# david-m-rosen/Optimization

Measured on AMD Instinct MI355X. Metric: TNT Steihaug-CG HVP+inner-product throughput, higher is better.
Workload: dtype f64

## Files before the change

include/mi355opt.h:

```cpp
#ifndef MI355OPT_H
#define MI355OPT_H

#include <stddef.h>
#include <stdint.h>

#ifdef __cplusplus
extern "C" {
#endif

#define MI_API __attribute__((visibility("default")))

typedef enum mi_status {
  MI_OK = 0,
  MI_ERR_INVALID_ARGUMENT = 1,
  MI_ERR_HIP = 2,
  MI_ERR_OOM = 3,
  MI_ERR_NO_DEVICE = 4,
  MI_ERR_COMM = 5,
  MI_ERR_INTERNAL = 6,
  MI_DECLINED = 7
} mi_status;

typedef struct mi_ctx mi_ctx;
typedef struct mi_vec mi_vec;
// ... 196 lines not shown
MI_API int mi_stiefel_retract(mi_ctx *ctx, size_t n, int p, const mi_vec *X, const mi_vec *V,
                              mi_vec *Y);
MI_API int mi_stiefel_rq_create(mi_ctx *ctx, const mi_csr *A, size_t n, int p, mi_stiefel_rq **out);
MI_API int mi_stiefel_rq_destroy(mi_stiefel_rq *prob);
MI_API int mi_stiefel_rq_objective(mi_stiefel_rq *prob, const mi_vec *X, double *f);
MI_API int mi_stiefel_rq_model(mi_stiefel_rq *prob, const mi_vec *X, mi_vec *grad, mi_op **hess);
MI_API int mi_stiefel_rq_trial(mi_stiefel_rq *prob, const mi_vec *X, const mi_vec *h, const mi_vec *g,
                               mi_vec *X_trial, double out[5]);
MI_API int mi_stiefel_rq_armijo_trial(mi_stiefel_rq *prob, const mi_vec *X, const mi_vec *g, double t, mi_vec *h_out,
                                      mi_vec *X_trial, double out[2]);
MI_API int mi_stiefel_rq_precon(mi_stiefel_rq *prob, const mi_vec *X, const mi_vec *dinv_rows,
                                mi_precon **out);

MI_API int mi_so3n_create(mi_ctx *ctx, size_t N, size_t n_edges, const int32_t *ei,
                          const int32_t *ej, const double *Rt , const double *w,
                          mi_so3n **out);
MI_API int mi_so3n_destroy(mi_so3n *prob);
MI_API int mi_so3n_objective(mi_so3n *prob, const mi_vec *R, double *f);
MI_API int mi_so3n_model(mi_so3n *prob, const mi_vec *R, mi_vec *grad, mi_op **hess,
                         mi_precon **block_jacobi );
MI_API int mi_so3n_retract(mi_so3n *prob, const mi_vec *R, const mi_vec *xi, mi_vec *Y);
MI_API int mi_so3n_trial(mi_so3n *prob, const mi_vec *R, const mi_vec *h, const mi_vec *g, int with_precon,
                         mi_vec *R_trial, double out[6]);

MI_API int mi_lobpcg_gram(mi_ctx *ctx, size_t m, int ka, int kb, const mi_vec *S, const mi_vec *AS,
                          double *G_host);
MI_API int mi_lobpcg_gram_split(mi_ctx *ctx, size_t m, int k, const mi_vec *S, int k1, const mi_vec *T1,
                                const mi_vec *T2, double *G_host);
MI_API int mi_lobpcg_gram_pair(mi_ctx *ctx, size_t m, int k, const mi_vec *S, int k1a, const mi_vec *Ta1,
                               const mi_vec *Ta2, int k1b, const mi_vec *Tb1, const mi_vec *Tb2, double *Ga_host,
                               double *Gb_host);
MI_API int mi_lobpcg_gram_pair_sym(mi_ctx *ctx, size_t m, int k, const mi_vec *S, int k1a, const mi_vec *Ta1,
                                   const mi_vec *Ta2, double *Ga_host, double *Gb_host);
typedef struct mi_panel_blocks {
  int nblocks;
  const mi_vec *block[3];
  int cols[3];
} mi_panel_blocks;
MI_API int mi_lobpcg_gram_pair_sym_blocks(mi_ctx *ctx, size_t m, const mi_panel_blocks *S, int k1a, const mi_vec *Ta1,
                                          const mi_vec *Ta2, double *Ga_host, double *Gb_host);
MI_API int mi_lobpcg_gram_pair_sym_tblocks(mi_ctx *ctx, size_t m, const mi_panel_blocks *S, const mi_panel_blocks *T,
                                           double *Ga_host, double *Gb_host);
MI_API int mi_lobpcg_gram_pair_gen_blocks(mi_ctx *ctx, size_t m, const mi_panel_blocks *S, const mi_panel_blocks *AS,
                                          const mi_panel_blocks *BS, double *Ga_host, double *Gb_host);
MI_API int mi_lobpcg_update2_blocks(mi_ctx *ctx, size_t m, const mi_panel_blocks *S, int kc, const double *C_host,
                                    int ldc, mi_vec *Y, int k1, mi_vec *Y2);
MI_API int mi_csr_spmm_colmajor_blocks(const mi_csr *A, const mi_panel_blocks *X, mi_vec *Y);
MI_API int mi_lobpcg_update(mi_ctx *ctx, size_t m, int ks, int kc, const mi_vec *S,
                            const double *C_host, int ldc, mi_vec *Y);
MI_API int mi_lobpcg_update2(mi_ctx *ctx, size_t m, int ks, int kc, const mi_vec *S, const double *C_host, int ldc,
                             mi_vec *Y, int k1, mi_vec *Y2);
MI_API int mi_lobpcg_residual(mi_ctx *ctx, size_t m, int nx, const mi_vec *AX, const mi_vec *BX,
                              const mi_vec *X, const double *theta_host, mi_vec *R, double *rnorm,
                              double *xnorm);
MI_API int mi_rayleigh_ritz(int n, const double *A, const double *B, double *Theta, double *C);
MI_API int mi_rayleigh_ritz_lowest(int n, int k, const double *A, const double *B, double *Theta, double *C);
MI_API int mi_csr_spmm_colmajor(const mi_csr *A, int k, const mi_vec *X, mi_vec *Y);
MI_API int mi_csr_spmm_colmajor_residual(const mi_csr *A, int nx, const mi_vec *X, const double *theta_host,
                                         mi_vec *AX, mi_vec *R, double *rnorm, double *xnorm);
MI_API int mi_panel_rowscale(mi_ctx *ctx, size_t m, int k, const mi_vec *d, const mi_vec *X, mi_vec *Y);

#define MI_COMM_UID_BYTES 128
MI_API int mi_comm_unique_id(unsigned char uid[MI_COMM_UID_BYTES]);
MI_API int mi_comm_init(mi_ctx *ctx, int world_size, int rank,
                        const unsigned char uid[MI_COMM_UID_BYTES]);
MI_API int mi_comm_finalize(mi_ctx *ctx);
MI_API int mi_comm_info(mi_ctx *ctx, int *world_size, int *rank);
MI_API int mi_comm_rccl_count(mi_ctx *ctx, int *nranks);
#define MI_COMM_IPC_HANDLE_BYTES 64
MI_API int mi_comm_ipc_export(mi_ctx *ctx, unsigned char handle[MI_COMM_IPC_HANDLE_BYTES]);
MI_API int mi_comm_ipc_attach(mi_ctx *ctx, int world_size, int rank,
                              const unsigned char *handles );
MI_API int mi_comm_ipc_selftest(mi_ctx *ctx, int *ok);
MI_API int mi_comm_ipc_enable(mi_ctx *ctx, int on);
MI_API int mi_comm_ipc_error(mi_ctx *ctx, int *err);
MI_API int mi_comm_ipc_fold(mi_ctx *ctx, int on);
MI_API int mi_comm_kernel_launches(mi_ctx *ctx, unsigned long long out[4]);
MI_API int mi_debug_csr_window_info(const mi_csr *A, size_t out[4]);
MI_API int mi_debug_csr_format_info(const mi_csr *A, size_t out[5]);
MI_API int mi_debug_so3n_info(const mi_so3n *q, size_t out[6]);
MI_API int mi_debug_window_runs(int ntiles, int max_wgs, int num_cu, size_t far_stride, int *bounds_out, int cap,
                                int *nb_out);
MI_API int mi_debug_stiefel_hess_form(int p, int gram_count, const size_t traits[9], const int switches[9], int out[14]);
MI_API int mi_debug_set_rank(mi_ctx *ctx, int world_size, int rank);
MI_API int mi_debug_csr_set_halo(mi_csr *A, int p, const double *halo_rows_host);
MI_API int mi_debug_time_fused_apply(mi_op *op, const mi_vec *in, mi_vec *out, int reps, double *us_per_call);
MI_API int mi_csr_shard_plan(size_t n_global, int world_size, int rank, const size_t *row_starts,
                             size_t nnz_local, const int64_t *col_global, int32_t *col_local, size_t *need_lo,
                             size_t *need_hi);
MI_API int mi_csr_create_sharded(mi_ctx *ctx, size_t n_global, size_t row_begin, size_t row_end,
                                 size_t nnz_local, const int32_t *rowptr, const int64_t *col_global,
                                 const double *val, const size_t *row_starts ,
                                 mi_csr **out);

#ifdef __cplusplus
}
#endif
#endif
```

optimization_amd/capi.py:

```python
import ctypes as C
import os

import numpy as np

_HERE = os.path.dirname(os.path.abspath(__file__))
LIB_PATH = os.environ.get("MI355OPT_LIB") or os.path.join(_HERE, "libmi355opt.so")

MI_OK = 0
STATUS = {0: "MI_OK", 1: "MI_ERR_INVALID_ARGUMENT", 2: "MI_ERR_HIP", 3: "MI_ERR_OOM",
          4: "MI_ERR_NO_DEVICE", 5: "MI_ERR_COMM", 6: "MI_ERR_INTERNAL", 7: "MI_DECLINED"}
KERNELS = ["none", "cg_init", "cg_dot3", "cg_scalar_a", "cg_update", "cg_scalar_b", "cg_pupdate",
           "csr_spmm", "stiefel_spmm_gram", "stiefel_gram_reduce", "stiefel_finish_dots",
           "stiefel_retract", "bsr3_spmv_dots", "blas1", "lobpcg_gram", "lobpcg_update",
           "lobpcg_residual", "stiefel_hess_fused", "comm_allreduce", "comm_halo"]
KID = {k: i for i, k in enumerate(KERNELS)}
STPCG_EXIT = ["RESIDUAL", "MAXIT", "KERNEL", "BOUNDARY", "USER"]

c_double_p = C.POINTER(C.c_double)
c_int32_p = C.POINTER(C.c_int32)
c_int64_p = C.POINTER(C.c_int64)
c_size_p = C.POINTER(C.c_size_t)
vp = C.c_void_p

APPLY_FN = C.CFUNCTYPE(C.c_int, vp, vp, vp)
# ... 121 lines not shown
        "mi_op_create_callback": [vp, C.c_size_t, APPLY_FN, vp, C.POINTER(vp)],
        "mi_op_create_callback_rect": [vp, C.c_size_t, C.c_size_t, APPLY_FN, vp, C.POINTER(vp)],
        "mi_op_create_callback_fused": [vp, C.c_size_t, APPLY_FN, APPLY_FUSED_FN, vp, C.POINTER(vp)],
        "mi_lsqr_default_params": [C.POINTER(LsqrParams)],
        "mi_lsqr": [vp, vp, vp, vp, C.POINTER(LsqrParams), vp, C.POINTER(LsqrResult)],
        "mi_op_create_diag": [vp, vp, C.POINTER(vp)],
        "mi_op_create_csr": [vp, vp, C.c_int, C.POINTER(vp)],
        "mi_op_apply": [vp, vp, vp],
        "mi_op_dims": [vp, c_size_p, c_size_p],
        "mi_op_destroy": [vp],
        "mi_precon_create_callback": [vp, C.c_size_t, APPLY_FN, vp, C.POINTER(vp)],
        "mi_precon_create_diag": [vp, vp, C.POINTER(vp)],
        "mi_precon_create_block3": [vp, vp, C.POINTER(vp)],
        "mi_precon_apply": [vp, vp, vp],
        "mi_precon_create_constraint": [vp, C.c_size_t, C.c_size_t, vp, vp, C.POINTER(vp)],
        "mi_precon_create_constraint_csr": [vp, C.c_size_t, C.c_size_t, c_int32_p, c_int32_p, c_double_p, vp, C.c_double,
                                            C.c_size_t, C.POINTER(vp)],
        "mi_precon_constraint_info": [vp, c_size_p, c_double_p, c_double_p, C.POINTER(C.c_int)],
        "mi_precon_constraint_solve": [vp, vp, vp, vp],
        "mi_precon_constraint_At": [vp, vp, vp],
        "mi_precon_destroy": [vp],
        "mi_stpcg": [vp, vp, vp, vp, C.POINTER(StpcgParams), vp, C.POINTER(StpcgResult),
                     C.POINTER(StpcgTrace)],
        "mi_stpcg_observed": [vp, vp, vp, vp, C.POINTER(StpcgParams), OBSERVER_FN, vp, vp, C.POINTER(StpcgResult),
                              C.POINTER(StpcgTrace)],
        "mi_stpcg_observer_available": [vp, C.POINTER(C.c_char_p)],
        "mi_lsqr_observed": [vp, vp, vp, vp, C.POINTER(LsqrParams), LSQR_OBSERVER_FN, vp, vp, C.POINTER(LsqrResult)],
        "mi_lsqr_observer_available": [vp, C.POINTER(C.c_char_p)],
        "mi_stiefel_gram": [vp, C.c_size_t, C.c_int, vp, vp, c_double_p],
        "mi_stiefel_project": [vp, C.c_size_t, C.c_int, vp, vp, vp],
        "mi_stiefel_retract": [vp, C.c_size_t, C.c_int, vp, vp, vp],
        "mi_stiefel_rq_create": [vp, vp, C.c_size_t, C.c_int, C.POINTER(vp)],
        "mi_stiefel_rq_destroy": [vp],
        "mi_stiefel_rq_objective": [vp, vp, c_double_p],
        "mi_stiefel_rq_model": [vp, vp, vp, C.POINTER(vp)],
        "mi_stiefel_rq_trial": [vp, vp, vp, vp, vp, c_double_p],
        "mi_stiefel_rq_armijo_trial": [vp, vp, vp, C.c_double, vp, vp, c_double_p],
        "mi_stiefel_rq_precon": [vp, vp, vp, C.POINTER(vp)],
        "mi_so3n_create": [vp, C.c_size_t, C.c_size_t, c_int32_p, c_int32_p, c_double_p, c_double_p,
                           C.POINTER(vp)],
        "mi_so3n_destroy": [vp],
        "mi_so3n_objective": [vp, vp, c_double_p],
        "mi_so3n_model": [vp, vp, vp, C.POINTER(vp), C.POINTER(vp)],
        "mi_so3n_retract": [vp, vp, vp, vp],
        "mi_so3n_trial": [vp, vp, vp, vp, C.c_int, vp, c_double_p],
        "mi_stpcg_collect": [vp, C.POINTER(StpcgResult)],
        "mi_lobpcg_gram": [vp, C.c_size_t, C.c_int, C.c_int, vp, vp, c_double_p],
        "mi_lobpcg_update": [vp, C.c_size_t, C.c_int, C.c_int, vp, c_double_p, C.c_int, vp],
        "mi_lobpcg_update2": [vp, C.c_size_t, C.c_int, C.c_int, vp, c_double_p, C.c_int, vp, C.c_int, vp],
        "mi_lobpcg_residual": [vp, C.c_size_t, C.c_int, vp, vp, vp, c_double_p, vp, c_double_p,
                               c_double_p],
        "mi_rayleigh_ritz": [C.c_int, c_double_p, c_double_p, c_double_p, c_double_p],
        "mi_rayleigh_ritz_lowest": [C.c_int, C.c_int, c_double_p, c_double_p, c_double_p, c_double_p],
        "mi_csr_spmm_colmajor": [vp, C.c_int, vp, vp],
        "mi_csr_spmm_colmajor_residual": [vp, C.c_int, vp, c_double_p, vp, vp, c_double_p, c_double_p],
        "mi_lobpcg_gram_split": [vp, C.c_size_t, C.c_int, vp, C.c_int, vp, vp, c_double_p],
        "mi_debug_window_runs": [C.c_int, C.c_int, C.c_int, C.c_size_t, C.POINTER(C.c_int), C.c_int, C.POINTER(C.c_int)],
        "mi_lobpcg_gram_pair": [vp, C.c_size_t, C.c_int, vp, C.c_int, vp, vp, C.c_int, vp, vp, c_double_p, c_double_p],
        "mi_lobpcg_gram_pair_sym": [vp, C.c_size_t, C.c_int, vp, C.c_int, vp, vp, c_double_p, c_double_p],
        "mi_lobpcg_gram_pair_sym_blocks": [vp, C.c_size_t, vp, C.c_int, vp, vp, c_double_p, c_double_p],
        "mi_lobpcg_gram_pair_gen_blocks": [vp, C.c_size_t, vp, vp, vp, c_double_p, c_double_p],
        "mi_lobpcg_gram_pair_sym_tblocks": [vp, C.c_size_t, vp, vp, c_double_p, c_double_p],
        "mi_lobpcg_update2_blocks": [vp, C.c_size_t, vp, C.c_int, c_double_p, C.c_int, vp, C.c_int, vp],
        "mi_csr_spmm_colmajor_blocks": [vp, vp, vp],
        "mi_panel_rowscale": [vp, C.c_size_t, C.c_int, vp, vp, vp],
        "mi_vec_view": [vp, C.c_size_t, C.c_size_t, C.POINTER(vp)],
        "mi_comm_unique_id": [C.POINTER(C.c_ubyte)],
        "mi_comm_init": [vp, C.c_int, C.c_int, C.POINTER(C.c_ubyte)],
        "mi_comm_finalize": [vp],
        "mi_comm_info": [vp, C.POINTER(C.c_int), C.POINTER(C.c_int)],
        "mi_comm_rccl_count": [vp, C.POINTER(C.c_int)],
        "mi_comm_ipc_export": [vp, C.POINTER(C.c_ubyte)],
        "mi_comm_ipc_attach": [vp, C.c_int, C.c_int, C.POINTER(C.c_ubyte)],
        "mi_comm_ipc_selftest": [vp, C.POINTER(C.c_int)],
        "mi_comm_ipc_enable": [vp, C.c_int],
        "mi_comm_ipc_error": [vp, C.POINTER(C.c_int)],
        "mi_comm_kernel_launches": [vp, C.POINTER(C.c_ulonglong)],
        "mi_comm_ipc_fold": [vp, C.c_int],
        "mi_debug_csr_window_info": [vp, c_size_p],
        "mi_debug_csr_format_info": [vp, c_size_p],
        "mi_debug_so3n_info": [vp, c_size_p],
        "mi_debug_time_fused_apply": [vp, vp, vp, C.c_int, c_double_p],
        "mi_debug_set_rank": [vp, C.c_int, C.c_int],
        "mi_debug_csr_set_halo": [vp, C.c_int, c_double_p],
        "mi_csr_create_sharded": [vp, C.c_size_t, C.c_size_t, C.c_size_t, C.c_size_t, c_int32_p,
                                  c_int64_p, c_double_p, c_size_p, C.POINTER(vp)],
    }
    for name, args in sigs.items():
        fn = getattr(L, name)
        fn.restype = C.c_int
        fn.argtypes = args
    L.mi_stpcg_default_params.restype = None
    L.mi_lsqr_default_params.restype = None
    L.mi_stpcg_default_params.argtypes = [C.POINTER(StpcgParams)]
    _lib = L
    return L


class FusionCounters(C.Structure):
    _fields_ = [(k, C.c_ulonglong) for k in ("fused_stpcg_solves", "generic_stpcg_solves", "fused_lsqr_solves",
                                             "generic_lsqr_solves", "fused_trial_steps", "generic_trial_steps",
                                             "generic_inner_products")]


def check(status):
    if status != MI_OK:
        raise MiError(status, load().mi_last_error().decode())


def window_runs(ntiles, max_wgs, num_cu=256, far_stride=0):
    L = load()
    cap = max(ntiles, max_wgs, 1) + 2
    buf = (C.c_int * cap)()
    nb = C.c_int(0)
    check(L.mi_debug_window_runs(ntiles, max_wgs, num_cu, far_stride, buf, cap, C.byref(nb)))
    return np.array(buf[:nb.value + 1], dtype=np.int64)


def stiefel_hess_form_fn():
    fn = load().mi_debug_stiefel_hess_form
    fn.restype = C.c_int
    fn.argtypes = [C.c_int, C.c_int, C.POINTER(C.c_size_t), C.POINTER(C.c_int), C.POINTER(C.c_int)]
    return fn


def stiefel_hess_form(p, gram_count, traits, switches):
    out = (C.c_int * 14)()
    st = stiefel_hess_form_fn()(p, gram_count, (C.c_size_t * 9)(*traits), (C.c_int * 9)(*switches), out)
    return list(out) if st == MI_OK else None


def csr_shard_plan(n_global, world_size, rank, row_starts, col_global):
    L = load()
    L.mi_csr_shard_plan.restype = C.c_int
    L.mi_csr_shard_plan.argtypes = [C.c_size_t, C.c_int, C.c_int, c_size_p, C.c_size_t, c_int64_p, c_int32_p,
                                    c_size_p, c_size_p]
    col_global = np.ascontiguousarray(col_global, dtype=np.int64)
    starts = (C.c_size_t * len(row_starts))(*[int(x) for x in row_starts])
    col_local = np.zeros(col_global.size, dtype=np.int32)
    lo, hi = C.c_size_t(0), C.c_size_t(0)
    check(L.mi_csr_shard_plan(n_global, world_size, rank, starts, col_global.size,
                              col_global.ctypes.data_as(c_int64_p), col_local.ctypes.data_as(c_int32_p),
                              C.byref(lo), C.byref(hi)))
    return col_local, lo.value, hi.value


def device_count():
    n = C.c_int(0)
    check(load().mi_device_count(C.byref(n)))
    return n.value


def _dp(a):
    return a.ctypes.data_as(c_double_p)


class Context:
    def __init__(self, device=0):
        self.L = load()
        self.h = vp()
        check(self.L.mi_ctx_create(device, C.byref(self.h)))

    def close(self):
        if self.h:
            self.L.mi_ctx_destroy(self.h)
            self.h = vp()

    def __enter__(self):
        return self

    def __exit__(self, *a):
        self.close()

    def sync(self):
        check(self.L.mi_ctx_sync(self.h))

    def set_option(self, name, value):
        check(self.L.mi_ctx_set_option(self.h, name.encode(), int(value)))
        return self

    def sync_count(self):
        n = C.c_size_t(0)
        check(self.L.mi_ctx_sync_count(self.h, C.byref(n)))
        return n.value

    def fusion_counters(self, reset=False):
        fc = FusionCounters()
        check(self.L.mi_ctx_fusion_counters(self.h, C.byref(fc)))
        if reset:
            check(self.L.mi_ctx_fusion_counters_reset(self.h))
        return {k: int(getattr(fc, k)) for k, _ in FusionCounters._fields_}

    def device_name(self):
        buf = C.create_string_buffer(256)
        check(self.L.mi_ctx_device_name(self.h, buf, 256))
        return buf.value.decode()

    def vec(self, n):
        return Vec(self, n)

    def upload(self, arr):
        arr = np.ascontiguousarray(arr, dtype=np.float64).ravel()
        v = Vec(self, arr.size)
        check(self.L.mi_vec_upload(v.h, _dp(arr), arr.size))
        return v

    def dot_batch(self, xs, ys):
        k = len(xs)
        X = (vp * k)(*[x.h for x in xs])
        Y = (vp * k)(*[y.h for y in ys])
        out = np.zeros(k)
        check(self.L.mi_vec_dot_batch(self.h, k, X, Y, _dp(out)))
        return out

    def timer_start(self):
        check(self.L.mi_timer_start(self.h))

    def timer_stop(self):
        ms = C.c_double(0)
        check(self.L.mi_timer_stop(self.h, C.byref(ms)))
        return ms.value

    def range_push(self, name):
        check(self.L.mi_range_push(name.encode()))

    def range_pop(self):
        check(self.L.mi_range_pop())

    def ktime_enable(self, name, on=True):
        check(self.L.mi_ktime_enable(self.h, KID[name], int(on)))

    def ktime_reset(self):
        check(self.L.mi_ktime_reset(self.h))

    def ktime_read(self, name):
        n = C.c_size_t(0)
        ms = C.c_double(0)
        check(self.L.mi_ktime_read(self.h, KID[name], C.byref(n), C.byref(ms)))
        return n.value, ms.value

    def csr(self, n, rowptr, col, val):
        return Csr(self, n, rowptr, col, val)

    def csr_sharded(self, n_global, row_begin, row_end, rowptr, col_global, val, row_starts):
        A = Csr.__new__(Csr)
        A.ctx, A.L = self, self.L
        rowptr = np.ascontiguousarray(rowptr, dtype=np.int32)
        col_global = np.ascontiguousarray(col_global, dtype=np.int64)
        val = np.ascontiguousarray(val, dtype=np.float64)
        starts = (C.c_size_t * len(row_starts))(*[int(x) for x in row_starts])
        A.n, A.nnz = row_end - row_begin, int(rowptr[-1])
        A.h = vp()
        check(self.L.mi_csr_create_sharded(self.h, n_global, row_begin, row_end, A.nnz,
                                           rowptr.ctypes.data_as(c_int32_p),
                                           col_global.ctypes.data_as(c_int64_p), _dp(val), starts,
                                           C.byref(A.h)))
        return A

    def op_diag(self, d):
        h = vp()
        check(self.L.mi_op_create_diag(self.h, d.h, C.byref(h)))
        return Op(self, h, keep=[d])
# ... 677 lines not shown
```

optimization_amd/csrc/context.hip:

```cpp
#include "mi_internal.h"
#include <chrono>
#include <cstring>
#include <strings.h>
#include <unistd.h>

#include <dlfcn.h>

namespace mi {

static thread_local char g_err[1024] = "";

void set_error(const char *fmt, ...) {
  va_list ap;
  va_start(ap, fmt);
  vsnprintf(g_err, sizeof(g_err), fmt, ap);
  va_end(ap);
}

int hip_fail(hipError_t e, const char *what, const char *file, int line) {
  set_error("HIP error %d (%s) in %s at %s:%d", (int)e, hipGetErrorString(e), what, file, line);
  (void)hipGetLastError();
  if (e == hipErrorNoDevice || e == hipErrorInvalidDevice) return MI_ERR_NO_DEVICE;
  if (e == hipErrorOutOfMemory) return MI_ERR_OOM;
  return MI_ERR_HIP;
// ... 122 lines not shown
  if (!p) return;
  auto it = ctx->pool_all.find(p);
  if (it == ctx->pool_all.end()) return;
  ctx->pool_free.insert({it->second, p});
}

int stage_upload(mi_ctx *ctx, const void *src, size_t bytes, void *dst_dev) {
  MI_REQUIRE(bytes <= mi_ctx::kStageBytes, "staged upload of %zu bytes exceeds the slot size", bytes);
  const int slot = ctx->stage_next;
  ctx->stage_next = (slot + 1) % mi_ctx::kStageSlots;
  if (!ctx->stage_host[slot]) {
    MI_HIP(hipHostMalloc(&ctx->stage_host[slot], mi_ctx::kStageBytes, hipHostMallocDefault));
    MI_HIP(hipEventCreateWithFlags(&ctx->stage_ev[slot], hipEventDisableTiming));
  } else {
    MI_HIP(hipEventSynchronize(ctx->stage_ev[slot]));
  }
  memcpy(ctx->stage_host[slot], src, bytes);
  MI_HIP(hipMemcpyAsync(dst_dev, ctx->stage_host[slot], bytes, hipMemcpyHostToDevice, ctx->stream));
  MI_HIP(hipEventRecord(ctx->stage_ev[slot], ctx->stream));
  return MI_OK;
}

hipEvent_t event_get(mi_ctx *ctx) {
  if (!ctx->event_pool.empty()) {
    hipEvent_t e = ctx->event_pool.back();
    ctx->event_pool.pop_back();
    return e;
  }
  hipEvent_t e = nullptr;
  if (hipEventCreate(&e) != hipSuccess) return nullptr;
  return e;
}

KScope::KScope(mi_ctx *c, int kid) : ctx(c), id(kid) {
  if (ctx->ktime[id].enabled) {
    e0 = event_get(ctx);
    e1 = event_get(ctx);
    if (e0) (void)hipEventRecord(e0, ctx->stream);
  }
}
KScope::~KScope() {
  if (e0 && e1) {
    (void)hipEventRecord(e1, ctx->stream);
    ctx->ktime[id].pending.push_back({e0, e1});
  }
}

}

using namespace mi;

namespace {
struct OptionDesc {
  const char *name;
  int (*set)(mi_ctx *, long);
  bool integer = false;
};
#define OPT_BOOL(FN, FIELD) \
  int FN(mi_ctx *c, long v) { c->FIELD = v != 0; return MI_OK; }
OPT_BOOL(opt_force_slot_path, force_slot_path)
OPT_BOOL(opt_force_lockstep, force_lockstep)
OPT_BOOL(opt_no_dirgram, no_dirgram)
OPT_BOOL(opt_dirgram_direct, dirgram_direct)
OPT_BOOL(opt_force_uniform_grid, cfg.force_uniform_grid)
OPT_BOOL(opt_no_fold, cfg.no_fold)
OPT_BOOL(opt_halo_push_late, cfg.halo_push_late)
OPT_BOOL(opt_no_packed, cfg.no_packed)
OPT_BOOL(opt_no_window, cfg.no_window)
OPT_BOOL(opt_no_win_bounds, cfg.no_win_bounds)
OPT_BOOL(opt_no_far_computed, cfg.no_far_computed)
OPT_BOOL(opt_words16, cfg.words16)
OPT_BOOL(opt_no_spmm_stream, cfg.no_spmm_stream)
OPT_BOOL(opt_no_spmm_win, cfg.no_spmm_win)
OPT_BOOL(opt_no_spmm_sweep, cfg.no_spmm_sweep)
OPT_BOOL(opt_no_zero_copy, cfg.no_zero_copy)
OPT_BOOL(opt_no_polled_sync, cfg.no_polled_sync)
OPT_BOOL(opt_no_update_mfma, cfg.no_update_mfma)
OPT_BOOL(opt_halo_rprime, cfg.halo_rprime)
OPT_BOOL(opt_no_gram_half, cfg.no_gram_half)
OPT_BOOL(opt_so3_no_quat, cfg.so3_no_quat)
OPT_BOOL(opt_so3_no_rquat, cfg.so3_no_rquat)
OPT_BOOL(opt_early_s, cfg.early_s)
OPT_BOOL(opt_defer_s, cfg.defer_s)
OPT_BOOL(opt_no_fused_observer, cfg.no_fused_observer)
OPT_BOOL(opt_no_fused_lsqr_observer, cfg.no_fused_lsqr_observer)
OPT_BOOL(opt_no_update_pair, cfg.no_update_pair)
OPT_BOOL(opt_two_kernel_step, cfg.two_kernel_step)
OPT_BOOL(opt_warn_generic, warn_generic)
OPT_BOOL(opt_tall_prologue, cfg.tall_prologue)
#undef OPT_BOOL
int opt_max_grid(mi_ctx *c, long v) {
  c->max_grid = (int)std::min<long>(kMaxGrid, std::max<long>(1, v));
  return MI_OK;
}
int opt_wide_quad(mi_ctx *c, long v) {
  c->cfg.wide_quad = v < 0 ? -1 : v != 0;
  return MI_OK;
}
int opt_wide_window(mi_ctx *c, long v) {
  c->cfg.wide_window = v < 0 ? -1 : v != 0;
  return MI_OK;
}
int opt_so3_sort_nbr(mi_ctx *c, long v) {
  c->cfg.so3_sort_nbr = (int)v;
  return MI_OK;
}
int opt_sweep_zsegs(mi_ctx *c, long v) {
  c->cfg.sweep_zsegs = (int)std::max<long>(0, std::min<long>(v, 1024));
  return MI_OK;
}
int opt_reanchor(mi_ctx *c, long v) {
  c->cfg.reanchor = (int)std::max<long>(0, std::min<long>(v, 1 << 20));
  return MI_OK;
}
int opt_ipc_timeout_ms(mi_ctx *c, long v) {
  c->cfg.ipc_timeout_ms = std::max<long>(0, v);
  return MI_OK;
}
const OptionDesc kOptions[] = {
    {"FORCE_SLOT_PATH", opt_force_slot_path}, {"FORCE_LOCKSTEP", opt_force_lockstep},
    {"NO_DIRGRAM", opt_no_dirgram}, {"DIRGRAM_DIRECT", opt_dirgram_direct}, {"MAX_GRID", opt_max_grid, true},
    {"FORCE_UNIFORM_GRID", opt_force_uniform_grid}, {"IPC_TIMEOUT_MS", opt_ipc_timeout_ms, true},
    {"NO_FOLD", opt_no_fold}, {"HALO_PUSH_LATE", opt_halo_push_late}, {"NO_PACKED", opt_no_packed},
    {"NO_WINDOW", opt_no_window}, {"NO_WIN_BOUNDS", opt_no_win_bounds}, {"NO_FAR_COMPUTED", opt_no_far_computed},
    {"WORDS16", opt_words16}, {"NO_SPMM_STREAM", opt_no_spmm_stream}, {"NO_SPMM_WIN", opt_no_spmm_win},
    {"NO_SPMM_SWEEP", opt_no_spmm_sweep}, {"SWEEP_ZSEGS", opt_sweep_zsegs, true},
    {"NO_ZERO_COPY", opt_no_zero_copy}, {"NO_POLLED_SYNC", opt_no_polled_sync}, {"WIDE_QUAD", opt_wide_quad, true}, {"WIDE_WINDOW", opt_wide_window, true},
    {"NO_UPDATE_MFMA", opt_no_update_mfma}, {"HALO_RPRIME", opt_halo_rprime}, {"NO_GRAM_HALF", opt_no_gram_half}, {"SO3_NO_QUAT", opt_so3_no_quat}, {"SO3_NO_RQUAT", opt_so3_no_rquat}, {"EARLY_S", opt_early_s}, {"DEFER_S", opt_defer_s}, {"NO_FUSED_OBSERVER", opt_no_fused_observer}, {"NO_FUSED_LSQR_OBSERVER", opt_no_fused_lsqr_observer}, {"NO_UPDATE_PAIR", opt_no_update_pair}, {"TWO_KERNEL_STEP", opt_two_kernel_step}, {"SO3_SORT_NBR", opt_so3_sort_nbr, true},
    {"WARN_GENERIC", opt_warn_generic}, {"TALL_PROLOGUE", opt_tall_prologue}, {"REANCHOR", opt_reanchor, true},
};
bool option_value(const OptionDesc &o, const char *e, long *v) {
  char *end = nullptr;
  *v = strtol(e, &end, 0);
  if (end != e && *end == '\0') return true;
  if (o.integer) {
    fprintf(stderr, "[mi355opt] warning: MI355OPT_%s=\"%s\" is not an integer; ignored (the default stays)\n", o.name, e);
    return false;
  }
  *v = (!strcasecmp(e, "no") || !strcasecmp(e, "false") || !strcasecmp(e, "off")) ? 0 : 1;
  return true;
}
void config_from_env(mi_ctx *ctx) {
  for (const OptionDesc &o : kOptions) {
    char name[64];
    snprintf(name, sizeof(name), "MI355OPT_%s", o.name);
    long v = 0;
    if (const char *e = getenv(name))
      if (option_value(o, e, &v)) (void)o.set(ctx, v);
  }
  static bool warned = false;
  if (warned || !environ) return;
  warned = true;
  for (char **ep = environ; *ep; ++ep) {
    if (strncmp(*ep, "MI355OPT_", 9) != 0) continue;
    const char *nm = *ep + 9, *eq = strchr(nm, '=');
    const size_t len = eq ? (size_t)(eq - nm) : strlen(nm);
    bool known = false;
    for (const OptionDesc &o : kOptions) known |= strlen(o.name) == len && strncmp(o.name, nm, len) == 0;
    for (const char *h : {"LIB", "COMM", "BUILD_TAG", "EXTRA_CFLAGS", "NO_UNITY"})
      known |= strlen(h) == len && strncmp(h, nm, len) == 0;
    known |= len >= 6 && strncmp(nm, "BENCH_", 6) == 0;
    if (!known)
      fprintf(stderr, "[mi355opt] warning: environment variable MI355OPT_%.*s is not a switch of this build (removed "
                      "or misspelt?); it changes nothing\n", (int)len, nm);
  }
}
}

extern "C" {

const char *mi_version(void) { return "mi355opt 0.1.0 (gfx950)"; }
const char *mi_last_error(void) { return g_err; }
const char *mi_status_string(int s) {
  switch (s) {
    case MI_OK: return "ok";
    case MI_ERR_INVALID_ARGUMENT: return "invalid argument";
    case MI_ERR_HIP: return "HIP runtime error";
    case MI_ERR_OOM: return "out of device memory";
    case MI_ERR_NO_DEVICE: return "no MI355X/HIP device (no CPU fallback)";
    case MI_ERR_COMM: return "RCCL communicator error";
    case MI_ERR_INTERNAL: return "internal error";
    case MI_DECLINED: return "declined (nothing was done)";
  }
  return "unknown status";
}

static const char *kKernelNames[MI_K_COUNT] = {
    "none", "cg_init", "cg_dot3", "cg_scalar_a", "cg_update", "cg_scalar_b", "cg_pupdate",
    "csr_spmm", "stiefel_spmm_gram", "stiefel_gram_reduce", "stiefel_finish_dots",
    "stiefel_retract", "bsr3_spmv_dots", "blas1", "lobpcg_gram", "lobpcg_update",
    "lobpcg_residual", "stiefel_hess_fused", "comm_allreduce", "comm_halo"};
const char *mi_kernel_name(int id) {
  if (id < 0 || id >= MI_K_COUNT) return "?";
  return kKernelNames[id];
}

int mi_ctx_set_option(mi_ctx *ctx, const char *name, long value) {
  MI_REQUIRE(ctx && name, "null argument");
  if (strncmp(name, "MI355OPT_", 9) == 0) name += 9;
  for (const OptionDesc &o : kOptions)
    if (strcmp(o.name, name) == 0) return o.set(ctx, value);
  set_error("unknown option '%s'", name);
  return MI_ERR_INVALID_ARGUMENT;
}

int mi_device_count(int *count) {
  MI_REQUIRE(count, "count is null");
  int c = 0;
  hipError_t e = hipGetDeviceCount(&c);
  if (e != hipSuccess) {
    (void)hipGetLastError();
// ... 248 lines not shown
```

optimization_amd/csrc/mi_internal.h:

```cpp
#pragma once

#include <hip/hip_runtime.h>

#include <cstdarg>
#include <cstdint>
#include <cstdio>
#include <cstring>
#include <map>
#include <string>
#include <set>
#include <vector>

#include "mi355opt.h"

namespace mi {

constexpr int kWave = 64;
constexpr int kBlock = 1024;
constexpr int kWaves = kBlock / kWave;
constexpr int kMaxP = 8;
constexpr int kMaxGrid = 512;
constexpr int kMaxRows = 1024;
constexpr int kMaxComps = 64;
constexpr int kNumXCD = 8;
// ... 29 lines not shown
    case 3: { constexpr int P = 3; __VA_ARGS__; } break;            \
    case 4: { constexpr int P = 4; __VA_ARGS__; } break;            \
    case 5: { constexpr int P = 5; __VA_ARGS__; } break;            \
    case 6: { constexpr int P = 6; __VA_ARGS__; } break;            \
    case 7: { constexpr int P = 7; __VA_ARGS__; } break;            \
    case 8: { constexpr int P = 8; __VA_ARGS__; } break;            \
    default: set_error("p must be in [1,%d], got %d", kMaxP, p); return MI_ERR_INVALID_ARGUMENT; \
  }
#define DISPATCH_P4(p, ...)                                         \
  switch (p) {                                                      \
    case 1: { constexpr int P = 1; __VA_ARGS__; } break;            \
    case 2: { constexpr int P = 2; __VA_ARGS__; } break;            \
    case 3: { constexpr int P = 3; __VA_ARGS__; } break;            \
    case 4: { constexpr int P = 4; __VA_ARGS__; } break;            \
    default: set_error("internal: narrow-row kernel asked for p = %d", p); return MI_ERR_INTERNAL; \
  }
#define DISPATCH_3(x, NAME, A, B, C, ...)                   \
  switch (x) {                                              \
    case A: { constexpr int NAME = A; __VA_ARGS__; } break; \
    case B: { constexpr int NAME = B; __VA_ARGS__; } break; \
    default: { constexpr int NAME = C; __VA_ARGS__; } break; \
  }
#define DISPATCH_FLAG(x, NAME, ...)                       \
  if (x) { constexpr bool NAME = true; __VA_ARGS__; }     \
  else { constexpr bool NAME = false; __VA_ARGS__; }

struct HostStatus {
  volatile uint64_t word;
  volatile uint32_t epoch;
};

struct CgState {
  double sk_M_pk, sk_M_2, pk_M_2;
  double target_rk_norm;
  double rv;
  double alpha, beta, kappa, sigma;
  double skplus1_M_2;
  double M_norm;
  unsigned long long k;
  unsigned long long launches;
  int mode;
  int exit_reason;
  double alpha_prev;
};
static_assert(sizeof(CgState) <= 128, "the CG state is meant to fit one 128-byte line");
struct CgConst {
  double Delta, Delta_2, epsilon;
  unsigned long long max_iterations;
  unsigned long long rag0, rag_per;
};
enum CgMode { CG_RUN = 0, CG_KERNEL_PENDING = 1, CG_APPLY_SIGMA = 2, CG_DONE = 3 };

struct Config {
  bool force_uniform_grid = false;
  long ipc_timeout_ms = 0;
  bool no_fold = false;
  bool halo_push_late = false;
  bool no_packed = false;
  bool no_window = false;
  bool no_win_bounds = false;
  bool no_far_computed = false;
  bool words16 = false;
  bool no_spmm_stream = false;
  bool no_spmm_sweep = true;
  int sweep_zsegs = 0;
  bool no_spmm_win = false;
  bool no_zero_copy = false;
  int wide_quad = -1;
  int wide_window = -1;
  bool no_polled_sync = false;
  bool two_kernel_step = false;
  int reanchor = 25;
  bool no_update_pair = false;
  bool no_gram_half = false;
  bool no_update_mfma = false;
  bool halo_rprime = false;
  bool early_s = false;
  bool defer_s = true;
  bool no_fused_observer = false;
  bool no_fused_lsqr_observer = false;
  bool so3_no_rquat = false;
  bool so3_no_quat = false;
  int so3_sort_nbr = 0;
  bool tall_prologue = false;
};

struct KTimer {
  bool enabled = false;
  std::vector<std::pair<hipEvent_t, hipEvent_t>> pending;
  size_t launches = 0;
  double total_ms = 0;
};

}

struct mi_ctx {
  int device = -1;
  hipStream_t stream = nullptr;
  char device_name[128] = {0};
  int num_cu = 256;
  bool uniform_grid = false;
  int max_grid = 512;
  std::multimap<size_t, void *> pool_free;
  std::map<void *, size_t> pool_all;
  size_t pool_bytes = 0;
  void *control_slab = nullptr;
  double *partials = nullptr;
  double *partials_b = nullptr;
  double *partials2 = nullptr;
  double *partials_user = nullptr;
  double *scalars = nullptr;
  double *host_scalars = nullptr;
  mi::CgState *cg = nullptr;
  mi::CgState *cg1 = nullptr;
  mi::CgState *cg_host = nullptr;
  const double *twok_r = nullptr;
  const mi::CgState *cg_live = nullptr;
  hipEvent_t cg_deferred_ev = nullptr;
  bool cg_deferred = false;
  size_t cg_deferred_hvp = 0;
  bool cg_in_observer = false;
  bool lsqr_in_observer = false;
  unsigned long long cg_deferred_seq = 0;
  mi::HostStatus *status = nullptr;
  mi::HostStatus *status_dev = nullptr;
  double *trace_dev = nullptr;
  size_t trace_cap = 0;
  unsigned int epoch = 0;
  uint64_t vec_serial = 0;
  size_t host_syncs = 0;
  mi_fusion_counters fusion = {0, 0, 0, 0, 0, 0, 0};
  bool warn_generic = false;
  bool warned_generic[3] = {false, false, false};
  static constexpr int kStageSlots = 4;
  static constexpr size_t kStageBytes = 96 * 96 * sizeof(double);
  void *stage_host[kStageSlots] = {nullptr, nullptr, nullptr, nullptr};
  hipEvent_t stage_ev[kStageSlots] = {nullptr, nullptr, nullptr, nullptr};
  int stage_next = 0;
  void *readback_host = nullptr;
  size_t readback_bytes = 0;
  unsigned long long *poll_flag = nullptr;
  unsigned long long poll_seq = 0;
  int st_win_occ[4][2][2][2] = {};
  bool st_widewin_lds[5][2][2] = {};
  int spmm_win_occ[2][2][2][2] = {};
  mi::KTimer ktime[MI_K_COUNT];
  std::vector<hipEvent_t> event_pool;
  hipEvent_t t_start = nullptr, t_stop = nullptr;
  void *comm = nullptr;
  int world_size = 1, rank = 0;
  bool force_slot_path = false;
  bool force_lockstep = false;
  bool no_dirgram = false;
  bool dirgram_direct = false;
  mi::Config cfg;
};

struct mi_vec {
  mi_ctx *ctx;
  size_t n;
  double *d;
  bool owned;
  uint64_t serial = 0;
  uint64_t gen = 0;
  mi_vec *root = nullptr;
  uint32_t views = 0;
  bool zombie = false;
};
namespace mi {
inline void touch(mi_vec *v) {
  if (v) ++(v->root ? v->root : v)->gen;
}
inline uint64_t gen_of(const mi_vec *v) { return (v->root ? v->root : v)->gen; }
}

namespace mi {

int pool_alloc(mi_ctx *ctx, size_t bytes, void **out);
void pool_free(mi_ctx *ctx, void *p);
int stage_upload(mi_ctx *ctx, const void *src, size_t bytes, void *dst_dev);
int readback_sync(mi_ctx *ctx, int n, const void *const *dev, const size_t *bytes, void *const *host);
int readback_area(mi_ctx *ctx, size_t bytes, void **host, void **dev);
int stream_wait(mi_ctx *ctx, const char *what);
unsigned long long poll_begin(mi_ctx *ctx, unsigned long long **flag_dev);
int poll_finish(mi_ctx *ctx, unsigned long long seq, const char *what);
int ensure_device();

inline int uniform_grid(const mi_ctx *ctx, size_t blocks) {
  if (ctx->uniform_grid) return kMaxGrid;
  if (blocks < 1) blocks = 1;
  if (blocks > (size_t)ctx->max_grid) blocks = ctx->max_grid;
  return (int)blocks;
}

inline int grid_for(const mi_ctx *ctx, size_t n, int per_thread) {
  if (ctx->uniform_grid) return kMaxGrid;
  size_t blocks = (n + (size_t)kBlock * per_thread - 1) / ((size_t)kBlock * per_thread);
  if (blocks < 1) blocks = 1;
  if (blocks > (size_t)ctx->max_grid) blocks = ctx->max_grid;
  return (int)blocks;
// ... 187 lines not shown
  const unsigned base = (xcd < r) ? xcd * (q + 1) : r * (q + 1) + (xcd - r) * q;
  return base + idx;
}

}

struct mi_csr {
  mi_ctx *ctx = nullptr;
  size_t n = 0;
  size_t ncols = 0;
  size_t nnz = 0;
  bool symmetric = false;
  size_t padded = 0;
  size_t nslices = 0;
  long long *slice_ptr = nullptr;
  int *col = nullptr;
  double *val = nullptr;
  uint32_t *pk = nullptr;
  double *vtab = nullptr;
  int nvtab = 0;
  int vtab_zero = -1;
  int win_chunks = 0;
  int win_head = 0;
  uint32_t win_zero = 0;
  uint32_t *wk = nullptr;
  int32_t *wfar = nullptr;
  uint32_t *wk16 = nullptr;
  size_t win_far_stride = 0;
  size_t win_far_pure = 0;
  struct WinPlan {
    int *bounds = nullptr;
    int n = 0;
  };
  mutable std::map<int, WinPlan> win_plans;
  size_t halo_lo = 0, halo_hi = 0;
  size_t send_lo = 0, send_hi = 0;
  double *halo = nullptr;
  bool halo_in_arena = false;
  size_t halo_off = 0, peer_lo_rows = 0;
  size_t halo_stride = 0;
  mutable unsigned long long halo_exchanges = 0;
  const double *halo_cur() const { return halo ? halo + (halo_exchanges & 1) * halo_stride : nullptr; }
  mutable double *halo_r = nullptr;
  mutable bool halo_r_in_arena = false;
  mutable size_t halo_r_off = 0;
  mutable unsigned long long halo_r_exchanges = 0;
};

namespace mi {
inline bool csr_row_sharded(const mi_csr *A) { return A->halo_lo + A->halo_hi + A->send_lo + A->send_hi > 0; }
inline bool far_computed(size_t win_far_pure, bool no_far_computed) {
  return win_far_pure > 0 && win_far_pure < ((size_t)1 << 31) && !no_far_computed;
}
inline bool csr_far_computed(const mi_ctx *ctx, const mi_csr *A) {
  return far_computed(A->win_far_pure, ctx->cfg.no_far_computed);
}
int csr_spmv_sub_scaled(const mi_csr *A, const mi_vec *V, const double *scale, const int *mode, const int *gate,
                        mi_vec *W, double *partials, int *nparts);
int csr_spmm_dots(const mi_csr *A, int p, const mi_vec *V, mi_vec *W, int *nparts, bool *unsupported);
int comm_halo_exchange(mi_ctx *ctx, const mi_csr *A, int p, const double *V);
int comm_exchange_halo_counts(mi_ctx *ctx, size_t need_lo, size_t need_hi, size_t *send_lo,
                              size_t *send_hi, size_t *peer_lo_rows, size_t *max_halo_rows);
int comm_halo_alloc(mi_ctx *ctx, size_t bytes, double **ptr, bool *in_arena, size_t *arena_off);
void comm_halo_free(mi_ctx *ctx, double *ptr, bool in_arena);
int csr_spmm_launch(const mi_csr *A, int p, const double *V, double *W);
int window_bounds(mi_ctx *ctx, const mi_csr *A, int wgs, int ntiles, int *grid, const int **bounds_out);
}

struct mi_op {
  mi_ctx *ctx = nullptr;
  size_t n = 0;
  size_t n_out = 0;
  int (*apply)(mi_op *self, const mi_vec *in, mi_vec *out) = nullptr;
  int (*apply_dots)(mi_op *self, const mi_vec *in, mi_vec *out, int *nparts) = nullptr;
  int (*apply_sub_scaled)(mi_op *self, const mi_vec *in, const double *scale, const int *mode, const int *gate,
                          mi_vec *inout, double *partials, int *nparts) = nullptr;
  const struct mi_dirgram *dirgram = nullptr;
  int (*apply_dir)(mi_op *self, const mi_vec *in, mi_vec *out, int gram_count, int *nparts) = nullptr;
  void (*destroy)(mi_op *self) = nullptr;
  void *impl = nullptr;
  bool borrowed = false;
};

struct mi_dirgram {
  int p = 0;
  size_t n = 0;
  const double *X = nullptr;
  const double *Y = nullptr;
  const double *S = nullptr;
  const struct mi_csr *halo_A = nullptr;
  bool twok = false;
};

struct mi_precon {
  mi_ctx *ctx = nullptr;
  size_t n = 0;
  int kind = 0;
  const double *data = nullptr;
  int (*apply)(mi_precon *self, const mi_vec *r, mi_vec *v) = nullptr;
  int (*apply_project)(mi_precon *self, mi_vec *r, mi_vec *v, int subtract) = nullptr;
  void (*destroy)(mi_precon *self) = nullptr;
  void *impl = nullptr;
  bool borrowed = false;
  double *fail_word = nullptr;
};
```

optimization_amd/csrc/stiefel.hip:

```cpp
#include "comm_ipc.h"
#include "spmm_core.h"
#include "stiefel_core.h"
#include "stiefel_tall.h"

#include <algorithm>
#include <cmath>
#include <cstdlib>
#include <vector>

using namespace mi;

namespace {

enum { POST_SYM = 1, POST_INVSQRT = 2 };

#ifndef MI_WIDE_NO_SCHED
#define MI_WIDE_SCHED() __builtin_amdgcn_sched_barrier(0)
#else
#define MI_WIDE_SCHED()
#endif
#ifndef MI_WIDE_CHUNK
#define MI_WIDE_CHUNK 2
#endif
#ifndef MI_WIDE_CHUNK_FROM
// ... 913 lines not shown
    }
#pragma unroll
    for (int a = 0; a < P; ++a)
#pragma unroll
      for (int b = 0; b < P; ++b) G[a * P + b] += x[a] * z[b];
  }
  if (SYM) store_sym_partials<P>(G, lds, partials);
  else block_partials_store_w<P * P, NW>(G, lds, partials);
}

template <int P, bool DOTS, bool FROM_SLOTS>
__global__ __launch_bounds__(StBlk<P>::threads) void k_st_finish(size_t n, const CgState *__restrict__ st,
                                                      const double *__restrict__ X,
                                                      const double *__restrict__ Z,
                                                      const double *__restrict__ Vin,
                                                      const double *__restrict__ gram_partials, int count,
                                                      const double *__restrict__ slots,
                                                      double *__restrict__ M_out,
                                                      double *__restrict__ out,
                                                      double *__restrict__ partials) {
  constexpr int BLK = StBlk<P>::threads, NW = StBlk<P>::waves;
  constexpr bool WIDE = P > 4;
  __shared__ double lds[SymIdx<P>::NS * (kWaves + 1) + 3 * kWaves];
  __shared__ double MmL[WIDE ? P * P : 1];
  if (st && st->mode != CG_RUN) return;
  const size_t stride = (size_t)gridDim.x * BLK;
  const size_t row0 = (size_t)blockIdx.x * BLK + threadIdx.x;
  double x[P], z[P], vi[P];
#pragma unroll
  for (int c = 0; c < P; ++c) { x[c] = 0; z[c] = 0; vi[c] = 0; }
  if (row0 < n) {
#pragma unroll
    for (int c = 0; c < P; ++c) {
      x[c] = X[row0 * P + c];
      z[c] = Z[row0 * P + c];
      if (DOTS) vi[c] = Vin[row0 * P + c];
    }
  }
  double Mm[P * P];
  load_sym<P, FROM_SLOTS>(gram_partials, count, slots, Mm, lds);
  if (M_out && blockIdx.x == 0 && threadIdx.x == 0) {
#pragma unroll
    for (int i = 0; i < P * P; ++i) M_out[i] = Mm[i];
  }
  if (WIDE) {
    if (threadIdx.x == 0) {
#pragma unroll
      for (int i = 0; i < P * P; ++i) MmL[i] = Mm[i];
    }
    __syncthreads();
  }
  double a[3] = {0, 0, 0};
  for (size_t row = row0; row < n;) {
    const size_t rnext = row + stride;
    double xn[P], zn[P], vn[P];
#pragma unroll
    for (int c = 0; c < P; ++c) { xn[c] = x[c]; zn[c] = z[c]; vn[c] = vi[c]; }
    if (rnext < n) {
#pragma unroll
      for (int c = 0; c < P; ++c) {
        xn[c] = X[rnext * P + c];
        zn[c] = Z[rnext * P + c];
        if (DOTS) vn[c] = Vin[rnext * P + c];
      }
    }
    if (WIDE) asm volatile("" ::: "memory");
#pragma unroll
    for (int b = 0; b < P; ++b) {
      double t = 0;
#pragma unroll
      for (int aa = 0; aa < P; ++aa) t += x[aa] * (WIDE ? MmL[aa * P + b] : Mm[aa * P + b]);
      const double o = z[b] - t;
      out[row * P + b] = o;
      if (DOTS) { a[0] += vi[b] * o; a[1] += o * o; a[2] += vi[b] * vi[b]; }
      if (WIDE) MI_WIDE_SCHED();
    }
    row = rnext;
#pragma unroll
    for (int c = 0; c < P; ++c) { x[c] = xn[c]; z[c] = zn[c]; vi[c] = vn[c]; }
  }
  if (DOTS) block_partials_store_w<3, NW>(a, lds, partials);
}

template <int P, bool FROM_SLOTS>
__global__ __launch_bounds__(StBlk<P>::threads) void k_st_polar(size_t n, double *__restrict__ Y,
                                                     const double *__restrict__ gram_partials, int count,
                                                     const double *__restrict__ slots) {
  constexpr int BLK = StBlk<P>::threads;
  constexpr bool WIDE = P > 4;
  __shared__ double lds[SymIdx<P>::NS * (kWaves + 1)];
  __shared__ double Minv[P * P];
  __shared__ double jac[WIDE ? 4 * P * P : 1];
  double G[P * P];
  load_sym<P, FROM_SLOTS>(gram_partials, count, slots, G, lds);
  if (WIDE) {
    if (threadIdx.x == 0) {
#pragma unroll
      for (int i = 0; i < P * P; ++i) jac[i] = G[i];
    }
    __syncthreads();
    if (threadIdx.x < 64) dev_sym_invsqrt_wave<P>(jac, jac + P * P, Minv);
  } else {
    if (threadIdx.x == 0) dev_sym_invsqrt<P>(G, Minv);
  }
  __syncthreads();
  double Mm[WIDE ? 1 : P * P];
  if (!WIDE) {
#pragma unroll
    for (int i = 0; i < P * P; ++i) Mm[i] = Minv[i];
  }
  const size_t stride = (size_t)gridDim.x * BLK;
  for (size_t row = (size_t)blockIdx.x * BLK + threadIdx.x; row < n; row += stride) {
    double y[P];
#pragma unroll
    for (int c = 0; c < P; ++c) y[c] = Y[row * P + c];
    if (WIDE) asm volatile("" ::: "memory");
#pragma unroll
    for (int b = 0; b < P; ++b) {
      double t = 0;
#pragma unroll
      for (int a = 0; a < P; ++a) t += y[a] * (WIDE ? Minv[a * P + b] : Mm[WIDE ? 0 : a * P + b]);
      Y[row * P + b] = t;
    }
  }
}

inline int row_grid(const mi_ctx *ctx, size_t n) { return grid_for(ctx, n, 2); }
inline int row_grid(const mi_ctx *ctx, size_t n, int p) {
  if (p <= 4 || ctx->uniform_grid) return row_grid(ctx, n);
  size_t blocks = std::max<size_t>(1, (n + 511) / 512);
  blocks = std::min<size_t>(blocks, std::min<size_t>(kMaxRows, 2 * (size_t)ctx->max_grid));
  return (int)blocks;
}
inline int nsym(int p) { return p * (p + 1) / 2; }

int sharded_reduce(mi_ctx *ctx, int count, int k, double *slots) {
  return reduce_rows_allreduce(ctx, ctx->partials2, count, k, slots);
}

int launch_spmm_gram(mi_ctx *ctx, const mi_csr *A, int p, const CgState *st, const double *V,
                     const double *X, const double *S, double *Z, int *count) {
  if (tall_p(p)) return tall_spmm_gram(ctx, A, p, st, V, X, S, Z, count);
  const size_t ngroups = sell_groups(A);
  int grid = uniform_grid(ctx, ngroups);
  MI_TRY(comm_halo_exchange(ctx, A, p, V));
  SellView view = sell_view(A);
  KScope ks(ctx, MI_K_STIEFEL_SPMM_GRAM);
  const bool no_stream = ctx->cfg.no_spmm_stream;
  MI_REQUIRE(p <= 4 || sell_stream_ok(A, p), "Stiefel rows of %d doubles need fields below 4 GiB", p);
  if ((!no_stream || p > 4) && sell_stream_ok(A, p)) {
    if (!ctx->uniform_grid && grid > 256) grid = 256;
    if (p > 4 && !ctx->uniform_grid)
      grid = (int)std::max<size_t>(1, std::min<size_t>((A->nslices + 3) / 4, std::min<size_t>(2 * (size_t)ctx->num_cu, 2 * (size_t)ctx->max_grid)));
    DISPATCH_FLAG(A->halo != nullptr, HL, DISPATCH_FLAG(A->pk != nullptr, PK, DISPATCH_P(p,
        hipLaunchKernelGGL((k_st_spmm_gram_stream<P, HL, PK>), dim3(grid), dim3(StBlk<P>::threads), 0, ctx->stream, view, st,
                           V, X, S, Z, ctx->partials2))));
  } else {
    DISPATCH_P4(p, hipLaunchKernelGGL(k_st_spmm_gram<P>, dim3(grid), dim3(kBlock), 0, ctx->stream, view, st, V,
                                      X, S, Z, ctx->partials2));
  }
  *count = grid;
  return MI_OK;
}

int launch_finish(mi_ctx *ctx, size_t n, int p, const CgState *st, const double *X, const double *Z,
                  const double *Vin, int count, double *M_out, double *out, bool dots, int *nparts) {
  if (tall_p(p)) return tall_finish(ctx, n, p, st, X, Z, Vin, count, M_out, out, dots, nparts);
  const int grid = row_grid(ctx, n, p);
  double *slots = ctx->scalars + SLOT_GRAM;
  const bool sharded = slot_mode(ctx);
  if (rows_mode(ctx)) MI_TRY(comm_allreduce_rows(ctx, ctx->partials2, nsym(p)));
  if (sharded) MI_TRY(sharded_reduce(ctx, count, nsym(p), slots));
  KScope ks(ctx, MI_K_STIEFEL_FINISH_DOTS);
  DISPATCH_FLAG(dots, D, DISPATCH_FLAG(sharded, F, DISPATCH_P(p,
      hipLaunchKernelGGL((k_st_finish<P, D, F>), dim3(grid), dim3(StBlk<P>::threads), 0, ctx->stream, n, st, X, Z, Vin,
                         (const double *)ctx->partials2, count, (const double *)slots, M_out, out, ctx->partials))));
  if (nparts) *nparts = grid;
  MI_HIP(hipGetLastError());
  return MI_OK;
}

int check_np(mi_ctx *ctx, size_t n, int p, const mi_vec *a, const mi_vec *b, const mi_vec *c) {
  MI_REQUIRE(ctx, "ctx is null");
  MI_REQUIRE(p >= 1 && p <= kMaxPTall, "p must be in [1,%d], got %d", kMaxPTall, p);
  if (tall_p(p)) MI_TRY(tall_check(ctx, nullptr, n, p));
  const mi_vec *vs[3] = {a, b, c};
  for (const mi_vec *v : vs) {
    if (!v) continue;
    MI_REQUIRE(v->ctx == ctx, "vector belongs to another context");
    MI_REQUIRE(v->n == n * (size_t)p, "expected an n x p = %zu x %d field, got %zu doubles", n, p, v->n);
  }
  return MI_OK;
}

}

struct mi_stiefel_rq {
  mi_ctx *ctx;
  const mi_csr *A;
  size_t n;
  int p;
  double *S_dev;
  mi_vec *Z;
  mi_vec *Y;
  mi_dirgram dg;
  mi_op hess;
  const mi_vec *X;
  uint64_t X_serial = 0;
  bool bound_to(const mi_vec *x) const { return X == x && x && X_serial == x->serial; }
  double *S_next = nullptr;
  mi_vec *Y_next = nullptr, *grad_next = nullptr, *Hh = nullptr;
  const mi_vec *trial_X = nullptr;
  const double *trial_d = nullptr;
  uint64_t trial_serial = 0, trial_gen = 0;
  bool warned_unsymmetric = false;
  void remember_trial(const mi_vec *Xt) {
    trial_X = Xt;
    trial_d = Xt->d;
    trial_serial = Xt->serial;
    trial_gen = gen_of(Xt);
  }
  bool is_trial(const mi_vec *X) const {
    return trial_X == X && trial_d == X->d && trial_serial == X->serial && trial_gen == gen_of(X);
  }
};

namespace {

int rq_apply_common(mi_op *self, const mi_vec *in, mi_vec *out, bool dots, int *nparts) {
  mi_stiefel_rq *q = (mi_stiefel_rq *)self->impl;
  mi_ctx *ctx = q->ctx;
  int count = 0;
  MI_TRY(launch_spmm_gram(ctx, q->A, q->p, ctx->cg_live, in->d, q->X->d, q->S_dev, q->Z->d, &count));
  return launch_finish(ctx, q->n, q->p, ctx->cg_live, q->X->d, q->Z->d, in->d, count, nullptr, out->d, dots,
                       nparts);
}
int rq_apply(mi_op *self, const mi_vec *in, mi_vec *out) {
  return rq_apply_common(self, in, out, false, nullptr);
}
int rq_apply_dots(mi_op *self, const mi_vec *in, mi_vec *out, int *nparts) {
  return rq_apply_common(self, in, out, true, nparts);
}

enum StHessForm {
  ST_HESS_PLAIN = 0,
  ST_HESS_WINDOW = 1,
  ST_HESS_WIDEWIN = 2,
  ST_HESS_WIDE = 3,
  ST_HESS_WIDEQ = 4
};

struct StHessTraits {
  bool pk, wk, wk16;
  int win_chunks, win_head;
  size_t win_far_pure, win_far_stride;
  bool halo, row_sharded;
  bool no_window, no_far_computed, words16, no_win_bounds, uniform_grid, slot_mode, twok_r;
  int wide_quad, wide_window;
};
StHessTraits st_hess_traits(const mi_ctx *ctx, const mi_csr *A) {
  const Config &c = ctx->cfg;
  return {A->pk != nullptr, A->wk != nullptr, A->wk16 != nullptr, A->win_chunks, A->win_head, A->win_far_pure,
          A->win_far_stride, A->halo != nullptr, csr_row_sharded(A), c.no_window, c.no_far_computed, c.words16,
          c.no_win_bounds, ctx->uniform_grid, slot_mode(ctx), ctx->twok_r != nullptr, c.wide_quad, c.wide_window};
}

struct StHessPlan {
  int form = ST_HESS_PLAIN;
  bool from_slots = false, halo = false, recur = false, pk = false, twok = false;
  int hw = 0;
  int far = 0;
  int block = kBlock;
  size_t lds_bytes = 0;
  int wc = 0;
  bool fard = false;
  bool run_table = false;
  bool exchange = false;
  bool gram_reduce = false;
  const char *error = nullptr;
};

int st_hess_plan(int p, int gram_count, const StHessTraits &t, StHessPlan *out) {
  StHessPlan &pl = *out = StHessPlan();
  const auto fail = [&](const char *why) { pl.error = why; return (int)MI_ERR_INVALID_ARGUMENT; };
  if (p < 1 || p > kMaxP) return fail("internal: the one-pass Hessian exists for rows of 1 ... 8 doubles");
  pl.fard = far_computed(t.win_far_pure, t.no_far_computed);
  const int hw = t.win_head <= 7 ? 7 : 8;
  const bool wide_window = (t.wide_window < 0 ? p <= 7 && !(t.wide_quad > 0) : t.wide_window != 0) && t.pk && t.wk &&
// ... 224 lines not shown
int mi_stiefel_gram(mi_ctx *ctx, size_t n, int p, const mi_vec *X, const mi_vec *Z, double *G_host) {
  MI_TRY(check_np(ctx, n, p, X, Z, nullptr));
  MI_REQUIRE(X && Z && G_host, "null argument");
  if (tall_p(p)) {
    int count = 0;
    MI_TRY(tall_gram(ctx, n, p, 0, false, X->d, Z->d, nullptr, nullptr, &count));
    MI_TRY(tall_reduce(ctx, count));
    double G[kTallTile];
    const void *dev[1] = {tall_reduced_row(ctx)};
    const size_t bytes[1] = {sizeof(G)};
    void *host[1] = {G};
    MI_TRY(readback_sync(ctx, 1, dev, bytes, host));
    for (int a = 0; a < p; ++a)
      for (int b = 0; b < p; ++b) G_host[a * p + b] = G[a * 16 + b];
    return MI_OK;
  }
  const int grid = row_grid(ctx, n, p);
  DISPATCH_P(p, hipLaunchKernelGGL((k_st_gram<P, 0, false>), dim3(grid), dim3(StBlk<P>::threads), 0, ctx->stream, n,
                                   (const double *)X->d, (const double *)Z->d, (const double *)nullptr,
                                   (double *)nullptr, ctx->partials2));
  double *slots = ctx->scalars + SLOT_RAW;
  MI_TRY(reduce_rows_allreduce(ctx, ctx->partials2, grid, p * p, slots));
  return read_slots_sync(ctx, SLOT_RAW, p * p, G_host);
}

int mi_stiefel_project(mi_ctx *ctx, size_t n, int p, const mi_vec *X, const mi_vec *Z, mi_vec *out) {
  MI_TRY(check_np(ctx, n, p, X, Z, out));
  MI_REQUIRE(X && Z && out, "null argument");
  touch(out);
  if (tall_p(p)) {
    int count = 0;
    MI_TRY(tall_gram(ctx, n, p, 0, true, X->d, Z->d, nullptr, nullptr, &count));
    return launch_finish(ctx, n, p, nullptr, X->d, Z->d, nullptr, count, nullptr, out->d, false, nullptr);
  }
  const int grid = row_grid(ctx, n, p);
  DISPATCH_P(p, hipLaunchKernelGGL((k_st_gram<P, 0, true>), dim3(grid), dim3(StBlk<P>::threads), 0, ctx->stream, n,
                                   (const double *)X->d, (const double *)Z->d, (const double *)nullptr,
                                   (double *)nullptr, ctx->partials2));
  return launch_finish(ctx, n, p, nullptr, X->d, Z->d, nullptr, grid, nullptr, out->d, false, nullptr);
}

int mi_stiefel_retract(mi_ctx *ctx, size_t n, int p, const mi_vec *X, const mi_vec *V, mi_vec *Y) {
  MI_TRY(check_np(ctx, n, p, X, V, Y));
  MI_REQUIRE(X && V && Y, "null argument");
  touch(Y);
  const int grid = row_grid(ctx, n, p);
  KScope ks(ctx, MI_K_STIEFEL_RETRACT);
  if (tall_p(p)) {
    int count = 0;
    MI_TRY(tall_gram(ctx, n, p, 1, true, X->d, V->d, nullptr, Y->d, &count));
    return tall_polar(ctx, n, p, Y->d, count);
  }
  DISPATCH_P(p, hipLaunchKernelGGL((k_st_gram<P, 1, true>), dim3(grid), dim3(StBlk<P>::threads), 0, ctx->stream, n,
                                   (const double *)X->d, (const double *)V->d, (const double *)nullptr,
                                   Y->d, ctx->partials2));
  double *slots = ctx->scalars + SLOT_GRAM;
  if (ctx->comm != nullptr || ctx->force_slot_path) {
    MI_TRY(sharded_reduce(ctx, grid, nsym(p), slots));
    DISPATCH_P(p, hipLaunchKernelGGL((k_st_polar<P, true>), dim3(grid), dim3(StBlk<P>::threads), 0, ctx->stream, n,
                                     Y->d, (const double *)ctx->partials2, grid, (const double *)slots));
  } else {
    DISPATCH_P(p, hipLaunchKernelGGL((k_st_polar<P, false>), dim3(grid), dim3(StBlk<P>::threads), 0, ctx->stream, n,
                                     Y->d, (const double *)ctx->partials2, grid, (const double *)slots));
  }
  MI_HIP(hipGetLastError());
  return MI_OK;
}

int mi_stiefel_rq_create(mi_ctx *ctx, const mi_csr *A, size_t n, int p, mi_stiefel_rq **out) {
  MI_REQUIRE(ctx && A && out, "null argument");
  MI_REQUIRE(p >= 1 && p <= kMaxPTall, "p must be in [1,%d], got %d", kMaxPTall, p);
  MI_REQUIRE(A->n == n && A->ctx == ctx, "matrix has %zu rows, expected %zu", A->n, n);
  if (tall_p(p)) MI_TRY(tall_check(ctx, A, n, p));
  mi_stiefel_rq *q = new mi_stiefel_rq();
  q->ctx = ctx;
  q->A = A;
  q->n = n;
  q->p = p;
  q->X = nullptr;
  MI_HIP(hipMalloc((void **)&q->S_dev, kMaxPTall * kMaxPTall * sizeof(double)));
  MI_HIP(hipMemsetAsync(q->S_dev, 0, kMaxPTall * kMaxPTall * sizeof(double), ctx->stream));
  MI_TRY(mi_vec_create(ctx, n * (size_t)p, &q->Z));
  MI_TRY(mi_vec_create(ctx, n * (size_t)p, &q->Y));
  q->hess.ctx = ctx;
  q->hess.n = n * (size_t)p;
  q->hess.apply = rq_apply;
  q->hess.apply_dots = rq_apply_dots;
  q->hess.apply_dir = rq_apply_dir;
  q->hess.impl = q;
  q->hess.borrowed = true;
  *out = q;
  return MI_OK;
}

int mi_stiefel_rq_destroy(mi_stiefel_rq *q) {
  if (!q) return MI_OK;
  (void)hipStreamSynchronize(q->ctx->stream);
  (void)hipFree(q->S_dev);
  (void)hipFree(q->S_next);
  mi_vec_destroy(q->Z);
  mi_vec_destroy(q->Y);
  mi_vec_destroy(q->Y_next);
  mi_vec_destroy(q->grad_next);
  mi_vec_destroy(q->Hh);
  delete q;
  return MI_OK;
}

int mi_stiefel_rq_objective(mi_stiefel_rq *q, const mi_vec *X, double *f) {
  MI_REQUIRE(q && X && f, "null argument");
  MI_TRY(check_np(q->ctx, q->n, q->p, X, nullptr, nullptr));
  mi_ctx *ctx = q->ctx;
  q->trial_X = nullptr;
  int count = 0;
  MI_TRY(launch_spmm_gram(ctx, q->A, q->p, nullptr, X->d, X->d, nullptr, q->Z->d, &count));
  if (tall_p(q->p)) {
    MI_TRY(tall_reduce(ctx, count));
    double Gt[kTallTile];
    const void *dev[1] = {tall_reduced_row(ctx)};
    const size_t bytes[1] = {sizeof(Gt)};
    void *host[1] = {Gt};
    MI_TRY(readback_sync(ctx, 1, dev, bytes, host));
    *f = tall_half_trace(Gt, q->p);
    return MI_OK;
  }
  double *slots = ctx->scalars + SLOT_GRAM;
  const int ns = nsym(q->p);
  MI_TRY(reduce_rows_allreduce(ctx, ctx->partials2, count, ns, slots));
  double G[kMaxP * (kMaxP + 1) / 2];
  MI_TRY(read_slots_sync(ctx, SLOT_GRAM, ns, G));
  double tr = 0;
  for (int a = 0, idx = 0; a < q->p; ++a) {
    tr += G[idx];
    idx += q->p - a;
  }
  *f = .5 * tr;
  return MI_OK;
}

int mi_stiefel_rq_model(mi_stiefel_rq *q, const mi_vec *X, mi_vec *grad, mi_op **hess) {
  MI_REQUIRE(q && X && grad, "null argument");
  MI_TRY(check_np(q->ctx, q->n, q->p, X, grad, nullptr));
  int count = 0;
  touch(grad);
  if (q->is_trial(X)) {
    std::swap(q->Y, q->Y_next);
    std::swap(q->S_dev, q->S_next);
    MI_TRY(mi_vec_copy(grad, q->grad_next));
  } else {
    MI_TRY(launch_spmm_gram(q->ctx, q->A, q->p, nullptr, X->d, X->d, nullptr, q->Y->d, &count));
    MI_TRY(launch_finish(q->ctx, q->n, q->p, nullptr, X->d, q->Y->d, nullptr, count, q->S_dev, grad->d, false,
                         nullptr));
  }
  q->trial_X = nullptr;
  q->X = X;
  q->X_serial = X->serial;
  q->dg.p = q->p;
  q->dg.n = q->n;
  q->dg.X = X->d;
  q->dg.Y = q->Y->d;
  q->dg.S = q->S_dev;
  q->dg.halo_A = q->A->halo ? q->A : nullptr;
  q->dg.twok = st_hess_twok_exists(q->p, st_hess_traits(q->ctx, q->A));
  q->hess.dirgram = (sell_stream_ok(q->A, q->p) && q->A->symmetric && !tall_p(q->p)) ? &q->dg : nullptr;
  if (!q->A->symmetric && !q->warned_unsymmetric) {
    q->warned_unsymmetric = true;
    fprintf(stderr, "mi355opt: the matrix of this Stiefel Rayleigh-quotient problem is not symmetric: the Hessian "
                    "operator keeps its two-pass form (P_X(A V - V S) with A as given)\n");
  }
  if (hess) *hess = &q->hess;
  return MI_OK;
}

int mi_stiefel_rq_trial(mi_stiefel_rq *q, const mi_vec *X, const mi_vec *h, const mi_vec *g, mi_vec *X_trial,
                        double out[5]) {
  MI_REQUIRE(q && X && h && g && X_trial && out, "null argument");
  MI_REQUIRE(q->bound_to(X), "mi_stiefel_rq_trial: the model is not bound to this X (call mi_stiefel_rq_model first)");
  MI_TRY(check_np(q->ctx, q->n, q->p, X, h, g));
  MI_TRY(check_np(q->ctx, q->n, q->p, X_trial, nullptr, nullptr));
  mi_ctx *ctx = q->ctx;
  ctx->fusion.fused_trial_steps++;
  const size_t N = q->n * (size_t)q->p;
  if (!q->Y_next) {
    MI_TRY(mi_vec_create(ctx, N, &q->Y_next));
    MI_TRY(mi_vec_create(ctx, N, &q->grad_next));
    MI_TRY(mi_vec_create(ctx, N, &q->Hh));
    MI_HIP(hipMalloc((void **)&q->S_next, kMaxPTall * kMaxPTall * sizeof(double)));
  }
  q->trial_X = nullptr;
  MI_TRY(rq_apply(&q->hess, h, q->Hh));
  {
    const double *xs[3] = {h->d, g->d, h->d}, *ys[3] = {h->d, h->d, q->Hh->d};
    MI_TRY(dot_batch_to_slots(ctx, 3, xs, ys, N, SLOT_MISC));
  }
  MI_TRY(mi_stiefel_retract(ctx, q->n, q->p, X, h, X_trial));
  int count = 0;
  MI_TRY(launch_spmm_gram(ctx, q->A, q->p, nullptr, X_trial->d, X_trial->d, nullptr, q->Y_next->d, &count));
  const int ns = nsym(q->p);
  const bool tall = tall_p(q->p);
  if (tall) MI_TRY(tall_reduce(ctx, count));
  else MI_TRY(reduce_rows_allreduce(ctx, ctx->partials2, count, ns, ctx->scalars + SLOT_GRAM));
  MI_TRY(launch_finish(ctx, q->n, q->p, nullptr, X_trial->d, q->Y_next->d, nullptr, tall ? 0 : count, q->S_next,
                       q->grad_next->d, false, nullptr));
  {
    const double *xs[1] = {q->grad_next->d}, *ys[1] = {q->grad_next->d};
    MI_TRY(dot_batch_to_slots(ctx, 1, xs, ys, N, SLOT_MISC + 3));
  }
  if (tall) {
    double Gt[kTallTile], misc[4];
    const void *dev[2] = {tall_reduced_row(ctx), ctx->scalars + SLOT_MISC};
    const size_t bytes[2] = {sizeof(Gt), sizeof(misc)};
    void *host[2] = {Gt, misc};
    MI_TRY(readback_sync(ctx, 2, dev, bytes, host));
    out[0] = tall_half_trace(Gt, q->p);
    for (int i = 0; i < 4; ++i) out[1 + i] = misc[i];
    q->remember_trial(X_trial);
    return MI_OK;
  }
  static_assert(SLOT_GRAM < SLOT_MISC && SLOT_MISC + 4 <= kScalarSlots, "slot map");
  double buf[SLOT_MISC + 4 - SLOT_GRAM];
  MI_TRY(read_slots_sync(ctx, SLOT_GRAM, SLOT_MISC + 4 - SLOT_GRAM, buf));
  double tr = 0;
  for (int a = 0, idx = 0; a < q->p; ++a) {
    tr += buf[idx];
    idx += q->p - a;
  }
  out[0] = .5 * tr;
  out[1] = buf[SLOT_MISC - SLOT_GRAM + 0];
  out[2] = buf[SLOT_MISC - SLOT_GRAM + 1];
  out[3] = buf[SLOT_MISC - SLOT_GRAM + 2];
  out[4] = buf[SLOT_MISC - SLOT_GRAM + 3];
  q->remember_trial(X_trial);
  return MI_OK;
}

int mi_stiefel_rq_armijo_trial(mi_stiefel_rq *q, const mi_vec *X, const mi_vec *g, double t, mi_vec *h_out,
                               mi_vec *X_trial, double out[2]) {
  MI_REQUIRE(q && X && g && h_out && X_trial && out, "null argument");
  MI_REQUIRE(q->bound_to(X),
             "mi_stiefel_rq_armijo_trial: the model is not bound to this X (call mi_stiefel_rq_model first)");
  MI_TRY(check_np(q->ctx, q->n, q->p, X, g, h_out));
  MI_TRY(check_np(q->ctx, q->n, q->p, X_trial, nullptr, nullptr));
  mi_ctx *ctx = q->ctx;
  ctx->fusion.fused_trial_steps++;
  const size_t N = q->n * (size_t)q->p;
  if (!q->Y_next) {
    MI_TRY(mi_vec_create(ctx, N, &q->Y_next));
    MI_TRY(mi_vec_create(ctx, N, &q->grad_next));
    MI_TRY(mi_vec_create(ctx, N, &q->Hh));
    MI_HIP(hipMalloc((void **)&q->S_next, kMaxPTall * kMaxPTall * sizeof(double)));
  }
  q->trial_X = nullptr;
  touch(X_trial);
  MI_TRY(mi_vec_scale_to(h_out, -t, g));
  MI_TRY(mi_stiefel_retract(ctx, q->n, q->p, X, h_out, X_trial));
  int count = 0;
  MI_TRY(launch_spmm_gram(ctx, q->A, q->p, nullptr, X_trial->d, X_trial->d, nullptr, q->Y_next->d, &count));
  const int ns = nsym(q->p);
  const bool tall = tall_p(q->p);
  if (tall) MI_TRY(tall_reduce(ctx, count));
  else MI_TRY(reduce_rows_allreduce(ctx, ctx->partials2, count, ns, ctx->scalars + SLOT_GRAM));
  MI_TRY(launch_finish(ctx, q->n, q->p, nullptr, X_trial->d, q->Y_next->d, nullptr, tall ? 0 : count, q->S_next,
                       q->grad_next->d, false, nullptr));
  {
    const double *xs[1] = {q->grad_next->d}, *ys[1] = {q->grad_next->d};
    MI_TRY(dot_batch_to_slots(ctx, 1, xs, ys, N, SLOT_MISC));
  }
  if (tall) {
    double Gt[kTallTile], misc[1];
    const void *dev[2] = {tall_reduced_row(ctx), ctx->scalars + SLOT_MISC};
    const size_t bytes[2] = {sizeof(Gt), sizeof(misc)};
    void *host[2] = {Gt, misc};
    MI_TRY(readback_sync(ctx, 2, dev, bytes, host));
    out[0] = tall_half_trace(Gt, q->p);
    out[1] = misc[0];
    q->remember_trial(X_trial);
    return MI_OK;
  }
  double buf[SLOT_MISC + 1 - SLOT_GRAM];
  MI_TRY(read_slots_sync(ctx, SLOT_GRAM, SLOT_MISC + 1 - SLOT_GRAM, buf));
  double tr = 0;
  for (int a = 0, idx = 0; a < q->p; ++a) {
    tr += buf[idx];
    idx += q->p - a;
  }
  out[0] = .5 * tr;
  out[1] = buf[SLOT_MISC - SLOT_GRAM];
  q->remember_trial(X_trial);
  return MI_OK;
}

int mi_stiefel_rq_precon(mi_stiefel_rq *q, const mi_vec *X, const mi_vec *dinv_rows, mi_precon **out) {
  MI_REQUIRE(q && X && dinv_rows && out, "null argument");
  MI_TRY(check_np(q->ctx, q->n, q->p, X, nullptr, nullptr));
  MI_REQUIRE(dinv_rows->n == q->n, "dinv_rows must have one entry per row");
  mi_precon *P = new mi_precon();
  P->ctx = q->ctx;
  P->n = q->n * (size_t)q->p;
  P->kind = 0;
  P->apply = rq_precon_apply;
  P->destroy = rq_precon_destroy;
  P->impl = new RqPreconImpl{q, X, dinv_rows};
  *out = P;
  return MI_OK;
}

}
```

optimization_amd/csrc/stpcg.hip:

```cpp
#include "comm_ipc.h"
#include "mi_internal.h"
#include "stiefel_core.h"

#include <cmath>
#include <type_traits>

using namespace mi;

namespace {

enum { PRE_NONE = 0, PRE_DIAG = 1, PRE_BLOCK3 = 2, PRE_EXTERNAL = 3 };

__device__ __forceinline__ void publish(HostStatus *hs, unsigned long long launches, int done) {
  __hip_atomic_store(&hs->word, (uint64_t)(launches << 1) | (uint64_t)(done ? 1 : 0), __ATOMIC_RELAXED,
                     __HIP_MEMORY_SCOPE_SYSTEM);
}

#define CG_FIELDS(X)                                                                               \
  X(sk_M_pk) X(sk_M_2) X(pk_M_2) X(target_rk_norm) X(rv) X(alpha) X(beta)                          \
  X(kappa) X(sigma) X(skplus1_M_2) X(M_norm) X(k) X(launches) X(mode) X(exit_reason)
__device__ __forceinline__ CgState load_state(const CgState *__restrict__ src) {
  CgState s;
#define X(f) s.f = src->f;
  CG_FIELDS(X)
// ... 97 lines not shown
      s[3 * b] = 0 * g0; s[3 * b + 1] = 0 * g1; s[3 * b + 2] = 0 * g2;
      v[3 * b] = v0; v[3 * b + 1] = v1; v[3 * b + 2] = v2;
      p[3 * b] = -v0; p[3 * b + 1] = -v1; p[3 * b + 2] = -v2;
      acc[0] += g0 * v0; acc[0] += g1 * v1; acc[0] += g2 * v2;
    }
  } else {
    const size_t n2 = n >> 1;
    for (size_t i = (size_t)blockIdx.x * kBlock + threadIdx.x; i < n2; i += stride) {
      const double2 gv = reinterpret_cast<const double2 *>(g)[i];
      reinterpret_cast<double2 *>(r)[i] = gv;
      reinterpret_cast<double2 *>(s)[i] = make_double2(0 * gv.x, 0 * gv.y);
      if (PRE == PRE_EXTERNAL) continue;
      double2 vv = gv;
      if (PRE == PRE_DIAG) {
        const double2 d = reinterpret_cast<const double2 *>(pre)[i];
        vv.x = d.x * gv.x; vv.y = d.y * gv.y;
        reinterpret_cast<double2 *>(v)[i] = vv;
      }
      reinterpret_cast<double2 *>(p)[i] = make_double2(-vv.x, -vv.y);
      acc[0] += gv.x * vv.x; acc[0] += gv.y * vv.y;
    }
    if ((n & 1) && blockIdx.x == 0 && threadIdx.x == 0) {
      const size_t i = n - 1;
      const double gv = g[i];
      r[i] = gv; s[i] = 0 * gv;
      if (PRE != PRE_EXTERNAL) {
        double vv = gv;
        if (PRE == PRE_DIAG) { vv = pre[i] * gv; v[i] = vv; }
        p[i] = -vv;
        acc[0] += gv * vv;
      }
    }
  }
  if (PRE == PRE_EXTERNAL) return;
  block_partials_store<1>(acc, lds, partials);
}

template <bool NEG_P>
__global__ __launch_bounds__(kBlock) void k_cg_dot_rv(size_t n, const CgState *__restrict__ st,
                                                      const double *__restrict__ r,
                                                      const double *__restrict__ v,
                                                      double *__restrict__ p,
                                                      double *__restrict__ partials) {
  __shared__ double lds[kWaves];
  if (!NEG_P && st->mode != CG_RUN) return;
  double acc[1] = {0};
  const size_t n2 = n >> 1, stride = (size_t)gridDim.x * kBlock;
  for (size_t i = (size_t)blockIdx.x * kBlock + threadIdx.x; i < n2; i += stride) {
    const double2 rv = reinterpret_cast<const double2 *>(r)[i];
    const double2 vv = reinterpret_cast<const double2 *>(v)[i];
    if (NEG_P) reinterpret_cast<double2 *>(p)[i] = make_double2(-vv.x, -vv.y);
    acc[0] += rv.x * vv.x; acc[0] += rv.y * vv.y;
  }
  if ((n & 1) && blockIdx.x == 0 && threadIdx.x == 0) {
    if (NEG_P) p[n - 1] = -v[n - 1];
    acc[0] += r[n - 1] * v[n - 1];
  }
  block_partials_store<1>(acc, lds, partials);
}

__global__ __launch_bounds__(kBlock) void k_cg_dot3(size_t n, const CgState *__restrict__ st,
                                                    const double *__restrict__ x,
                                                    const double *__restrict__ y,
                                                    double *__restrict__ partials) {
  __shared__ double lds[3 * kWaves];
  if (st && st->mode != CG_RUN) return;
  double a[3] = {0, 0, 0};
  const size_t n2 = n >> 1, stride = (size_t)gridDim.x * kBlock;
  for (size_t i = (size_t)blockIdx.x * kBlock + threadIdx.x; i < n2; i += stride) {
    const double2 xv = reinterpret_cast<const double2 *>(x)[i];
    const double2 yv = reinterpret_cast<const double2 *>(y)[i];
    a[0] += xv.x * yv.x; a[0] += xv.y * yv.y;
    a[1] += yv.x * yv.x; a[1] += yv.y * yv.y;
    a[2] += xv.x * xv.x; a[2] += xv.y * xv.y;
  }
  if ((n & 1) && blockIdx.x == 0 && threadIdx.x == 0) {
    const double xv = x[n - 1], yv = y[n - 1];
    a[0] += xv * yv; a[1] += yv * yv; a[2] += xv * xv;
  }
  block_partials_store<3>(a, lds, partials);
}

__device__ __forceinline__ void gdir_from_rows(const double *__restrict__ partials, int count, int gns,
                                               double *__restrict__ gdir) {
  const int lane = threadIdx.x & 63;
  for (int w = threadIdx.x >> 6; w < gns; w += kWaves) {
    const double *src = partials + (size_t)w * kMaxRows;
    double t[kMaxRows / 64];
#pragma unroll
    for (int j = 0; j < kMaxRows / 64; ++j) {
      const int r = lane + 64 * j;
      t[j] = (r < count) ? src[r] : 0.0;
    }
    double v = 0;
#pragma unroll
    for (int j = 0; j < kMaxRows / 64; ++j) v += t[j];
    v = wave_reduce_sum(v);
    if (lane == 0) {
      gdir[SLOT_GDIR_P + w] = v;
      gdir[w] = -v;
    }
  }
}

__device__ __forceinline__ void gdir_rows_to(const double *__restrict__ partials, int count, int gns,
                                             double *__restrict__ dst) {
  const int lane = threadIdx.x & 63;
  for (int w = threadIdx.x >> 6; w < gns; w += kWaves) {
    const double *src = partials + (size_t)w * kMaxRows;
    double t[kMaxRows / 64];
#pragma unroll
    for (int j = 0; j < kMaxRows / 64; ++j) {
      const int r = lane + 64 * j;
      t[j] = (r < count) ? src[r] : 0.0;
    }
    double v = 0;
#pragma unroll
    for (int j = 0; j < kMaxRows / 64; ++j) v += t[j];
    v = wave_reduce_sum(v);
    if (lane == 0) dst[w] = v;
  }
}

struct CgSetup {
  double Delta, kappa_fgr, theta, epsilon;
  unsigned long long max_iterations;
};

template <bool FROM_SLOTS>
__global__ __launch_bounds__(kBlock) void k_cg_scalar_init(CgState *st, CgSetup cfg,
                                                           const double *partials, int nparts,
                                                           const double *slots, HostStatus *hs,
                                                           const double *__restrict__ gpartials, int gcount, int gns,
                                                           double *__restrict__ gdir) {
#pragma clang fp contract(off)
  __shared__ double lds[kWaves + 1];
  if (gdir) gdir_from_rows(gpartials, gcount, gns, gdir);
  double red[1];
  if (FROM_SLOTS) red[0] = slots[0];
  else reduce_rows<1>(partials, nparts, red, lds);
  if (threadIdx.x != 0) return;
  CgState s;
  const double rv0 = red[0];
  s.sk_M_pk = 0;
  s.sk_M_2 = 0;
  s.pk_M_2 = rv0;
  const double r0_norm = sqrt(rv0);
  const double pw = pow(r0_norm, cfg.theta);
  s.target_rk_norm = r0_norm * ((pw < cfg.kappa_fgr) ? pw : cfg.kappa_fgr);
  s.rv = rv0;
  s.alpha = s.beta = s.kappa = s.sigma = s.skplus1_M_2 = 0;
  s.M_norm = 0;
  s.k = 0;
  s.launches = 0;
  s.exit_reason = MI_STPCG_EXIT_MAXIT;
  s.mode = CG_RUN;
  if (cfg.max_iterations == 0) {
    s.mode = CG_DONE;
    s.M_norm = sqrt(0.0);
  } else if (sqrt(rv0) <= s.target_rk_norm) {
    s.mode = CG_DONE;
    s.exit_reason = MI_STPCG_EXIT_RESIDUAL;
    s.M_norm = sqrt(0.0);
  }
  store_state(st, s);
  publish(hs, 0, s.mode == CG_DONE);
}

struct DirGramArgs {
  const double *X, *Y, *S;
  double *gpartials;
  double *gdir;
  int ns;
};

#ifdef MI_FOLD_STAMPS
}
extern "C" __attribute__((visibility("default"))) int mi_debug_fold_stamp_buffer(void *dev_ptr) {
  return (int)hipMemcpyToSymbol(HIP_SYMBOL(mi::g_fold_stamps), &dev_ptr, sizeof(dev_ptr));
}
namespace {
#endif

template <int SP>
struct DirGramLds {
  static constexpr int value = (SymIdx<SP>::NS * kWaves > kWaves + 1) ? SymIdx<SP>::NS * kWaves : kWaves + 1;
};
template <>
struct DirGramLds<0> {
  static constexpr int value = kWaves + 1;
};
static_assert(kWaves + 1 >= kIpcVals, "LDS of the folded exchange");

#define CG_KERNEL_ATTR
#define CG_UPDATE_SIGMA 1
#define CG_UPDATE_NAME k_cg_update
#define CG_PUPDATE_NAME k_cg_pupdate
#include "stpcg_kernels.inc"
#undef CG_KERNEL_ATTR
#undef CG_UPDATE_NAME
#undef CG_PUPDATE_NAME
#define CG_KERNEL_ATTR __attribute__((amdgpu_num_sgpr(80), amdgpu_waves_per_eu(8, 8)))
#define CG_UPDATE_NAME k_cg_update_s80
#define CG_PUPDATE_NAME k_cg_pupdate_s80
#include "stpcg_kernels.inc"
#undef CG_KERNEL_ATTR
#undef CG_UPDATE_NAME
#undef CG_PUPDATE_NAME
#undef CG_UPDATE_SIGMA
#define CG_UPDATE_SIGMA 0
#define CG_KERNEL_ATTR
#define CG_UPDATE_NAME k_cg_update_ns
#define CG_PUPDATE_NAME k_cg_pupdate_ns_unused
#include "stpcg_kernels.inc"
#undef CG_KERNEL_ATTR
#undef CG_UPDATE_NAME
#undef CG_PUPDATE_NAME
#define CG_KERNEL_ATTR __attribute__((amdgpu_num_sgpr(80), amdgpu_waves_per_eu(8, 8)))
#define CG_UPDATE_NAME k_cg_update_ns_s80
#define CG_PUPDATE_NAME k_cg_pupdate_ns_s80_unused
#include "stpcg_kernels.inc"
#undef CG_KERNEL_ATTR
#undef CG_UPDATE_NAME
#undef CG_PUPDATE_NAME
#undef CG_UPDATE_SIGMA

template <class F>
__device__ __forceinline__ void reduce_rows_1x512(const double *__restrict__ partials, int count, double &out, double *lds,
                                                  F &&after_issue) {
  const int lane = threadIdx.x & 63, w = threadIdx.x >> 6;
  double t[8];
#pragma unroll
  for (int j = 0; j < 8; ++j) t[j] = 0.0;
  if (w == 0) {
#pragma unroll
    for (int j = 0; j < 8; ++j) {
      const int r = lane + 64 * j;
      if (r < count) t[j] = partials[r];
    }
  }
  after_issue();
  if (w == 0) {
    double v = 0;
#pragma unroll
    for (int j = 0; j < 8; ++j) v += t[j];
    v = wave_reduce_sum(v);
    if (lane == 0) lds[0] = v;
  }
  __syncthreads();
  out = lds[0];
  __syncthreads();
}

__global__ __launch_bounds__(kBlock) __attribute__((amdgpu_waves_per_eu(8, 8))) void k_cg_pupdate_early(
    size_t n, CgConst cc, const CgState *__restrict__ st_in, CgState *__restrict__ st_out,
    const double *__restrict__ partials_b, int nparts_b, const double *__restrict__ v, double *__restrict__ p,
    double *__restrict__ s, HostStatus *hs, double *__restrict__ trace, size_t trace_cap, DirGramArgs dg) {
  __shared__ double lds[kWaves + 1];
  const unsigned n2 = (unsigned)(n >> 1), stride = gridDim.x * kBlock, i0 = blockIdx.x * kBlock + threadIdx.x;
  const unsigned tail0 = (unsigned)cc.rag0, per = (unsigned)cc.rag_per;
  const unsigned irem = (threadIdx.x < per) ? tail0 + blockIdx.x * per + threadIdx.x : n2;
  auto next_of = [&](unsigned i_) -> unsigned {
    const unsigned j_ = i_ + stride;
    return j_ < tail0 ? j_ : ((i_ < tail0 && irem < n2) ? irem : n2);
  };
  const unsigned ifirst = i0 < tail0 ? i0 : (irem < n2 ? irem : n2);
  unsigned Le[3];
  {
    unsigned L = ifirst;
#pragma unroll
    for (int j = 0; j < 3; ++j) {
      Le[j] = L;
      if (L < n2) L = next_of(L);
    }
  }
  double2 pe[3], ve[3], se[3];
  CgState cs = load_state(st_in);
  const bool leader = blockIdx.x == 0 && threadIdx.x == 0;
  if (cs.mode == CG_DONE) {
    if (leader) store_state(st_out, cs);
    return;
  }
  const int mode_in = cs.mode;
  auto early_s = [&] {
    if (mode_in != CG_RUN) return;
    const double alpha = cs.alpha;
#pragma unroll
    for (int j = 0; j < 3; ++j)
      if (Le[j] < n2) {
        pe[j] = reinterpret_cast<double2 *>(p)[Le[j]];
        se[j] = reinterpret_cast<double2 *>(s)[Le[j]];
      }
#pragma unroll
    for (int j = 0; j < 3; ++j)
      if (Le[j] < n2) ve[j] = reinterpret_cast<const double2 *>(v)[Le[j]];
#pragma unroll
    for (int j = 0; j < 3; ++j)
      if (Le[j] < n2) {
        double2 sv = se[j];
        const double2 pv = pe[j];
        sv.x = sv.x + alpha * pv.x; sv.y = sv.y + alpha * pv.y;
        reinterpret_cast<double2 *>(s)[Le[j]] = sv;
      }
  };
  double red = 0;
  if (mode_in != CG_APPLY_SIGMA) reduce_rows_1x512(partials_b, nparts_b, red, lds, early_s);
  step_b(cs, cc, red);
  cs.launches = cs.launches + 1;
// ... 70 lines not shown
      vv0 = reinterpret_cast<const double2 *>(v)[ifirst];
      pv0 = reinterpret_cast<const double2 *>(pc)[ifirst];
      if (FLUSH) {
        ov0 = reinterpret_cast<double2 *>(px)[ifirst];
        sv0 = reinterpret_cast<double2 *>(s)[ifirst];
      }
    }
  };
  double red[1] = {0};
  if (mode_in != CG_APPLY_SIGMA) reduce_rows<1>(partials_b, nparts_b, red, lds, prefetch_now);
  else prefetch_now();
  step_b(cs, cc, red[0]);
  cs.launches = cs.launches + 1;
  const bool dir = mode_in == CG_RUN && cs.mode == CG_RUN;
  if (leader) {
    store_state(st_out, cs);
    if (!FLUSH && dir) st_out->alpha_prev = cs.alpha;
    if (mode_in == CG_RUN && trace && cs.k - 1 < trace_cap) {
      const size_t k = (size_t)(cs.k - 1);
      trace[k] = cs.alpha;
      trace[trace_cap + k] = cs.beta;
      trace[2 * trace_cap + k] = cs.kappa;
      trace[3 * trace_cap + k] = cs.rv;
    }
    publish(hs, cs.launches, cs.mode == CG_DONE);
    if (dg.gdir && dir) {
      for (int i = 0; i < dg.ns; ++i) dg.gdir[SLOT_GDIR_P + i] = -dg.gdir[i] + cs.beta * dg.gdir[SLOT_GDIR_P + i];
    }
  }
  const double beta = cs.beta;
  if (FLUSH) {
    const double alpha_old = st_out->alpha_prev, alpha = mode_in == CG_RUN ? cs.alpha : cs.sigma;
    double2 vv = vv0, pv = pv0, ov = ov0, sv = sv0;
    for (size_t i = ifirst; i < n2;) {
      const size_t inext = next_of(i);
      double2 vn = vv, pn = pv, on = ov, sn = sv;
      if (inext < n2) {
        vn = reinterpret_cast<const double2 *>(v)[inext];
        pn = reinterpret_cast<const double2 *>(pc)[inext];
        on = reinterpret_cast<double2 *>(px)[inext];
        sn = reinterpret_cast<double2 *>(s)[inext];
      }
      sv.x = sv.x + alpha_old * ov.x; sv.y = sv.y + alpha_old * ov.y;
      sv.x = sv.x + alpha * pv.x; sv.y = sv.y + alpha * pv.y;
      reinterpret_cast<double2 *>(s)[i] = sv;
      if (dir) {
        pv.x = -vv.x + beta * pv.x; pv.y = -vv.y + beta * pv.y;
        reinterpret_cast<double2 *>(px)[i] = pv;
      }
      i = inext; vv = vn; pv = pn; ov = on; sv = sn;
    }
    if ((n & 1) && leader) {
      s[n - 1] = s[n - 1] + alpha_old * px[n - 1];
      s[n - 1] = s[n - 1] + alpha * pc[n - 1];
      if (dir) px[n - 1] = -v[n - 1] + beta * pc[n - 1];
    }
  } else if (dir) {
    double2 vv = vv0, pv = pv0;
    for (size_t i = ifirst; i < n2;) {
      const size_t inext = next_of(i);
      double2 vn = vv, pn = pv;
      if (inext < n2) {
        vn = reinterpret_cast<const double2 *>(v)[inext];
        pn = reinterpret_cast<const double2 *>(pc)[inext];
      }
      pv.x = -vv.x + beta * pv.x; pv.y = -vv.y + beta * pv.y;
      reinterpret_cast<double2 *>(px)[i] = pv;
      i = inext; vv = vn; pv = pn;
    }
    if ((n & 1) && leader) px[n - 1] = -v[n - 1] + beta * pc[n - 1];
  } else if (mode_in != CG_APPLY_SIGMA) {
    const double alpha = mode_in == CG_RUN ? cs.alpha : cs.sigma;
    for (size_t i = i0; i < n2; i += stride) {
      const double2 pv = reinterpret_cast<const double2 *>(pc)[i];
      double2 sv = reinterpret_cast<double2 *>(s)[i];
      sv.x = sv.x + alpha * pv.x; sv.y = sv.y + alpha * pv.y;
      reinterpret_cast<double2 *>(s)[i] = sv;
    }
    if ((n & 1) && leader) s[n - 1] = s[n - 1] + alpha * pc[n - 1];
  }
}


template <int NS>
__global__ __launch_bounds__(kBlock) void k_cg_step2(size_t n, CgConst cc, const CgState *__restrict__ st_in,
                                                     CgState *__restrict__ st_out, const double *__restrict__ partials_a,
                                                     int nparts_a, const double *__restrict__ Hp, double *__restrict__ r,
                                                     double *__restrict__ p, double *__restrict__ s, HostStatus *hs,
                                                     double *__restrict__ trace, size_t trace_cap, DirGramArgs dg) {
  constexpr int KC = 3 + NS + 2;
  __shared__ double lds[3 * (kWaves + 1)];
  static_assert(KC <= kWaves, "one wave per component");
  CgState cs = load_state(st_in);
  const bool leader = blockIdx.x == 0 && threadIdx.x == 0;
  if (cs.mode == CG_DONE) {
    if (leader) store_state(st_out, cs);
    return;
  }
  const size_t n2 = n >> 1, stride = (size_t)gridDim.x * kBlock, i0 = (size_t)blockIdx.x * kBlock + threadIdx.x;
  double2 hv0 = make_double2(0, 0), rv0 = hv0, pv0 = hv0, sv0 = hv0;
  auto prefetch = [&] {
    if (i0 < n2) {
      hv0 = reinterpret_cast<const double2 *>(Hp)[i0];
      rv0 = reinterpret_cast<double2 *>(r)[i0];
      pv0 = reinterpret_cast<double2 *>(p)[i0];
      sv0 = reinterpret_cast<double2 *>(s)[i0];
    }
  };
  double d[KC];
  reduce_rows<KC>(partials_a, nparts_a, d, lds, prefetch);
  step_a(cs, cc, d[0], d[1], d[2]);
  const int mode_a = cs.mode;
  double red = 0;
  {
#pragma clang fp contract(off)
    if (mode_a == CG_RUN) red = cs.rv + 2 * cs.alpha * d[KC - 2] + cs.alpha * cs.alpha * d[1];
    else if (mode_a == CG_KERNEL_PENDING) red = d[KC - 1];
  }
  step_b(cs, cc, red);
  cs.launches = cs.launches + 1;
  if (leader) {
    store_state(st_out, cs);
    if (mode_a == CG_RUN && trace && cs.k - 1 < trace_cap) {
      const size_t k = (size_t)(cs.k - 1);
      trace[k] = cs.alpha;
      trace[trace_cap + k] = cs.beta;
      trace[2 * trace_cap + k] = cs.kappa;
      trace[3 * trace_cap + k] = cs.rv;
    }
    publish(hs, cs.launches, cs.mode == CG_DONE);
    if (mode_a == CG_RUN) {
      for (int i = 0; i < NS; ++i) dg.gdir[i] = dg.gdir[i] + cs.alpha * d[3 + i];
      if (cs.mode == CG_RUN)
        for (int i = 0; i < NS; ++i) dg.gdir[SLOT_GDIR_P + i] = -dg.gdir[i] + cs.beta * dg.gdir[SLOT_GDIR_P + i];
    }
  }
  if (mode_a != CG_RUN) {
    const double sigma = cs.sigma;
    for (size_t i = i0; i < n2; i += stride) {
      const double2 pv = reinterpret_cast<const double2 *>(p)[i];
      double2 sv = reinterpret_cast<double2 *>(s)[i];
      sv.x += sigma * pv.x; sv.y += sigma * pv.y;
      reinterpret_cast<double2 *>(s)[i] = sv;
    }
    if ((n & 1) && leader) s[n - 1] += sigma * p[n - 1];
    return;
  }
  const double alpha = cs.alpha, beta = cs.beta;
  const bool dir = cs.mode == CG_RUN;
  double2 hv = hv0, rv = rv0, pv = pv0, sv = sv0;
  for (size_t i = i0; i < n2;) {
    const size_t inext = i + stride;
    double2 hn = hv, rn = rv, pn = pv, sn = sv;
    if (inext < n2) {
      hn = reinterpret_cast<const double2 *>(Hp)[inext];
      rn = reinterpret_cast<double2 *>(r)[inext];
      pn = reinterpret_cast<double2 *>(p)[inext];
      sn = reinterpret_cast<double2 *>(s)[inext];
    }
    rv.x += alpha * hv.x; rv.y += alpha * hv.y;
    reinterpret_cast<double2 *>(r)[i] = rv;
    sv.x = sv.x + alpha * pv.x; sv.y = sv.y + alpha * pv.y;
    reinterpret_cast<double2 *>(s)[i] = sv;
    if (dir) {
      pv.x = -rv.x + beta * pv.x; pv.y = -rv.y + beta * pv.y;
      reinterpret_cast<double2 *>(p)[i] = pv;
// ... 195 lines not shown
  const int grid = grid_for(ctx, n, 4);
  KScope ks(ctx, MI_K_CG_DOT3);
  hipLaunchKernelGGL(k_cg_dot3, dim3(grid), dim3(kBlock), 0, ctx->stream, n, ctx->cg_live, x, y,
                     ctx->partials);
  *nparts = grid;
  return MI_OK;
}
}

extern "C" {

void mi_stpcg_default_params(mi_stpcg_params *p) {
  if (!p) return;
  p->Delta = 1.0;
  p->max_iterations = 1000;
  p->kappa_fgr = .1;
  p->theta = .5;
  p->epsilon = 1e-8;
  p->run_ahead = 0;
  p->constraint_At = 0;
  p->defer_result = 0;
}

static inline double *precon_fail_host(mi_ctx *ctx) { return reinterpret_cast<double *>(ctx->cg_host + 1); }
static int precon_fail_check(mi_ctx *ctx, mi_stpcg_result *result) {
  const double w = *precon_fail_host(ctx);
  if (result) result->precon_status = (int)w;
  if (w != 1.0) return MI_OK;
  set_error("the preconditioner of this solve reported a failed application (code 1: its inner iteration broke down -- "
            "dependent constraint rows, or NaN / Inf in the residual): the result is not a projected step");
  return MI_ERR_INTERNAL;
}

__global__ void k_cg_result_to_host(unsigned long long *host, const unsigned long long *__restrict__ st,
                                    const double *__restrict__ fail_dev, unsigned long long *flag,
                                    unsigned long long seq) {
  constexpr int kWords = (int)(sizeof(CgState) / 8);
  static_assert(sizeof(CgState) % 8 == 0, "CgState is copied in 8-byte words");
  if (threadIdx.x < kWords) host[threadIdx.x] = st[threadIdx.x];
  if (threadIdx.x == kWords) reinterpret_cast<double *>(host)[kWords] = fail_dev ? *fail_dev : 0.0;
  __threadfence_system();
  __syncthreads();
  if (threadIdx.x == 0) __hip_atomic_store(flag, seq, __ATOMIC_RELEASE, __HIP_MEMORY_SCOPE_SYSTEM);
}
static unsigned long long result_to_host(mi_ctx *ctx, const CgState *st_final, const mi_precon *P) {
  unsigned long long *flag = nullptr, *hdev = nullptr;
  unsigned long long seq = poll_begin(ctx, &flag);
  if (!seq) return 0;
  if (hipHostGetDevicePointer((void **)&hdev, ctx->cg_host, 0) != hipSuccess) {
    (void)hipGetLastError();
    return 0;
  }
  hipLaunchKernelGGL(k_cg_result_to_host, dim3(1), dim3(64), 0, ctx->stream, hdev,
                     reinterpret_cast<const unsigned long long *>(st_final),
                     (const double *)(P ? P->fail_word : nullptr), flag, seq);
  if (hipGetLastError() != hipSuccess) return 0;
  return seq;
}

}

namespace {

#define DISPATCH_4(x, NAME, A, B, C, D, ...)                \
  switch (x) {                                              \
    case A: { constexpr int NAME = A; __VA_ARGS__; } break; \
    case B: { constexpr int NAME = B; __VA_ARGS__; } break; \
    case C: { constexpr int NAME = C; __VA_ARGS__; } break; \
    default: { constexpr int NAME = D; __VA_ARGS__; } break; \
  }
#define DISPATCH_PRE(pre, ...) DISPATCH_4(pre, PRE, PRE_NONE, PRE_DIAG, PRE_BLOCK3, PRE_EXTERNAL, __VA_ARGS__)
#define DISPATCH_KC(kc, ...) DISPATCH_4(kc, KC, 4, 6, 9, 16, __VA_ARGS__)
#define DISPATCH_KC_WIDE(kc, ...) DISPATCH_4(kc, KC, 18, 24, 31, 39, __VA_ARGS__)
#define DISPATCH_SP(sp, ...) \
  if ((sp) == 0) { constexpr int SP = 0; __VA_ARGS__; } else DISPATCH_4(sp, SP, 1, 2, 3, 4, __VA_ARGS__)

template <bool SIGMA, int KC>
auto cg_update_recur_kernel() {
  if constexpr (SIGMA && KC == 16) return &k_cg_update_s80<PRE_NONE, false, KC, NoFold>;
  else if constexpr (SIGMA) return &k_cg_update<PRE_NONE, false, KC, NoFold>;
  else if constexpr (KC == 16) return &k_cg_update_ns_s80<PRE_NONE, false, KC, NoFold>;
  else return &k_cg_update_ns<PRE_NONE, false, KC, NoFold>;
}
template <bool FS, int SP>
auto cg_pupdate_kernel() {
  if constexpr (SP == 1 || (FS && SP == 0)) return &k_cg_pupdate_s80<FS, SP, NoFold>;
  else return &k_cg_pupdate<FS, SP, NoFold>;
}

struct StpcgPlan {
  size_t n;
  bool observed, sharded, rows, lockstep, recur, folded, init_fused, gdir_in_scalar_init;
  bool twok, early, defer;
  int pre, run_ahead, grid, gns, sp, kc, reanchor;
  const mi_dirgram *dgp;
  CgConst cc;
};

int stpcg_plan(const mi_ctx *ctx, const mi_op *H, const mi_precon *P, const mi_stpcg_params *prm, size_t n,
               bool observed, StpcgPlan &pl) {
  pl.n = n;
  pl.observed = observed;
  pl.pre = !P ? PRE_NONE : (P->kind == 1 ? PRE_DIAG : (P->kind == 2 ? PRE_BLOCK3 : PRE_EXTERNAL));
  MI_REQUIRE(pl.pre != PRE_BLOCK3 || n % 3 == 0, "block-Jacobi preconditioner needs n divisible by 3");
  pl.sharded = slot_mode(ctx);
  pl.rows = rows_mode(ctx);
  pl.dgp = (!ctx->no_dirgram && H->dirgram && H->apply_dir) ? H->dirgram : nullptr;
  if (pl.dgp && pl.dgp->p > 4 && (pl.pre != PRE_NONE || ctx->dirgram_direct)) pl.dgp = nullptr;
  MI_REQUIRE(!pl.dgp || (pl.dgp->p >= 1 && pl.dgp->p <= kMaxP && pl.dgp->n * (size_t)pl.dgp->p == n),
             "operator's direction-Gram description does not match the problem dimension");
  pl.run_ahead = prm->run_ahead > 0 ? prm->run_ahead : 3;
  pl.lockstep = (ctx->comm != nullptr && ctx->world_size > 1) || ctx->force_lockstep;
  pl.grid = (pl.pre == PRE_BLOCK3) ? grid_for(ctx, n / 3, 2) : grid_for(ctx, n, 4);
  pl.cc = CgConst{prm->Delta, prm->Delta * prm->Delta, prm->epsilon, (unsigned long long)prm->max_iterations, 0ull, 0ull};
  const size_t n2 = n >> 1, step = (size_t)pl.grid * kBlock;
  pl.cc.rag0 = (n2 / step) * step;
  pl.cc.rag_per = (n2 - pl.cc.rag0 + (size_t)pl.grid - 1) / (size_t)pl.grid;
  pl.recur = pl.dgp && pl.pre == PRE_NONE && !ctx->dirgram_direct;
  pl.gns = pl.dgp ? pl.dgp->p * (pl.dgp->p + 1) / 2 : 0;
  pl.sp = (pl.dgp && !pl.recur) ? pl.dgp->p : 0;
  pl.kc = pl.recur ? dir_comps(pl.dgp->p) : 3;
  pl.folded = pl.sharded && pl.recur && pl.kc <= kIpcVals && comm_fold_enabled(ctx) && !ctx->force_slot_path;
  pl.init_fused = pl.recur && n == pl.dgp->n * (size_t)pl.dgp->p;
  pl.gdir_in_scalar_init = pl.recur && !pl.sharded && !pl.rows;
  pl.twok = ctx->cfg.two_kernel_step && pl.recur && pl.dgp->twok && pl.dgp->p == 3 && !pl.sharded && !pl.rows &&
            !pl.lockstep && pl.init_fused && pl.gdir_in_scalar_init && !observed;
  pl.early = !pl.sharded && !pl.rows && pl.sp == 0 && ctx->cfg.early_s && pl.grid <= 512 &&
             pl.cc.rag0 <= 2ull * (size_t)pl.grid * kBlock && (n >> 1) < ((size_t)1 << 31) && !observed;
  pl.defer = !pl.sharded && !pl.rows && !pl.lockstep && !pl.twok && pl.sp == 0 && !pl.early && ctx->cfg.defer_s &&
             !observed;
  pl.reanchor = (pl.recur && !pl.twok && ctx->cfg.reanchor > 0) ? ctx->cfg.reanchor : 0;
  return MI_OK;
}

struct StpcgBufs {
  mi_ctx *ctx;
  mi_vec *r = nullptr, *v = nullptr, *p = nullptr, *p2 = nullptr, *Hp = nullptr;
  bool ok = false;
  const mi_vec *g = nullptr; mi_vec *s_out = nullptr; mi_op *H = nullptr;
  mi_precon *P = nullptr; const mi_stpcg_params *prm = nullptr;
  double *vd = nullptr;
  const double *pred = nullptr;
  DirGramArgs dga{nullptr, nullptr, nullptr, nullptr, nullptr, 0};
  double *slots_g = nullptr, *slots_a = nullptr, *slots_b = nullptr;
  CgState *st0 = nullptr, *st1 = nullptr;
  double *tr = nullptr;
  size_t tcap = 0;
  bool rprime = false;
  unsigned long long *peek_dev = nullptr;
  explicit StpcgBufs(mi_ctx *c) : ctx(c) {}
  StpcgBufs(const StpcgBufs &) = delete;
  StpcgBufs &operator=(const StpcgBufs &) = delete;
  ~StpcgBufs() {
    ctx->cg_live = nullptr;
    comm_halo_fold_drop(ctx);
    if (!ok) (void)hipStreamSynchronize(ctx->stream);
    for (mi_vec *x : {r, p, p2, Hp, v}) mi_vec_destroy(x);
  }
};

int stpcg_bufs(mi_ctx *ctx, const StpcgPlan &pl, const mi_vec *g, mi_op *H, mi_precon *P, const mi_stpcg_params *prm,
               mi_vec *s_out, const mi_stpcg_trace *trace, StpcgBufs &b) {
  const size_t n = pl.n;
  b.g = g, b.s_out = s_out, b.H = H, b.P = P, b.prm = prm;
  MI_TRY(mi_vec_create(ctx, n, &b.r));
  MI_TRY(mi_vec_create(ctx, n, &b.p));
  MI_TRY(mi_vec_create(ctx, n, &b.Hp));
  if (pl.pre != PRE_NONE) MI_TRY(mi_vec_create(ctx, n, &b.v));
  if (pl.defer) MI_TRY(mi_vec_create(ctx, n, &b.p2));
  b.vd = (pl.pre == PRE_NONE) ? b.r->d : b.v->d;
  b.pred = P ? P->data : nullptr;
  if (trace && trace->cap) {
    if (ctx->trace_cap < trace->cap) {
      if (ctx->trace_dev) MI_HIP(hipFree(ctx->trace_dev));
      MI_HIP(hipMalloc((void **)&ctx->trace_dev, 4 * trace->cap * sizeof(double)));
      ctx->trace_cap = trace->cap;
    }
    b.tcap = ctx->trace_cap;
    b.tr = ctx->trace_dev;
  }
  if (pl.dgp)
    b.dga = DirGramArgs{pl.dgp->X, pl.dgp->Y, pl.dgp->S, ctx->partials2, pl.recur ? ctx->scalars + SLOT_GDIR : nullptr,
                        pl.gns};
  b.slots_g = ctx->scalars + SLOT_GRAM, b.slots_a = ctx->scalars + SLOT_CG, b.slots_b = ctx->scalars + SLOT_CG + 4;
  b.st0 = ctx->cg, b.st1 = ctx->cg1;
  if (pl.observed) {
    const hipError_t e = hipHostGetDevicePointer((void **)&b.peek_dev, ctx->cg_host, 0);
    if (e != hipSuccess) return hip_fail(e, "stpcg observer: device address of the pinned words", __FILE__, __LINE__);
  }
  return MI_OK;
}

int stpcg_allreduce(mi_ctx *ctx, const StpcgPlan &pl, double *partials, int count, int k, double *slots) {
  return pl.sharded ? reduce_rows_allreduce(ctx, partials, count, k, slots)
                    : pl.rows ? comm_allreduce_rows(ctx, partials, k) : MI_OK;
}

int launch_dirgram(mi_ctx *ctx, const StpcgPlan &pl, const StpcgBufs &b, const double *vec) {
  DISPATCH_P(pl.dgp->p, hipLaunchKernelGGL(k_cg_dirgram<P>, dim3(pl.grid), dim3(StBlk<P>::threads), 0, ctx->stream,
                                           pl.dgp->n, vec, b.dga));
  return MI_OK;
}
void launch_gdir_anchor(mi_ctx *ctx, const StpcgPlan &pl, const StpcgBufs &b, double *dst, double *dst2) {
  hipLaunchKernelGGL(k_cg_gdir_anchor, dim3(1), dim3(kBlock), 0, ctx->stream, (const double *)ctx->partials2, pl.grid,
                     pl.gns, (const double *)b.slots_g, pl.sharded ? 1 : 0, (const CgState *)b.st0, dst, dst2);
}
template <class K, class FOLD>
void launch_cg_update(K kernel, mi_ctx *ctx, const StpcgPlan &pl, const StpcgBufs &b, int nparts, const FOLD &fold) {
  hipLaunchKernelGGL(kernel, dim3(pl.grid), dim3(kBlock), 0, ctx->stream, pl.n, pl.cc, (const CgState *)b.st0, b.st1,
                     (const double *)ctx->partials, nparts, (const double *)(pl.recur ? b.slots_g : b.slots_a),
                     (const double *)b.p->d, (const double *)b.Hp->d, b.pred, b.s_out->d, b.r->d, b.vd, ctx->partials_b,
                     b.dga, fold);
}
template <class K, class FOLD>
void launch_cg_pupdate(K kernel, mi_ctx *ctx, const StpcgPlan &pl, const StpcgBufs &b, const FOLD &fold) {
  hipLaunchKernelGGL(kernel, dim3(pl.grid), dim3(kBlock), 0, ctx->stream, pl.n, pl.cc, (const CgState *)b.st1, b.st0,
                     (const double *)ctx->partials_b, pl.grid, (const double *)b.slots_b, (const double *)b.vd, b.p->d,
                     b.s_out->d, ctx->status_dev, b.tr, b.tcap, b.dga, fold);
}

int stpcg_precondition(mi_ctx *ctx, const StpcgPlan &pl, StpcgBufs &b, bool first) {
  mi_precon *P = b.P;
  if (P->apply_project) MI_TRY(P->apply_project(P, b.r, b.v, b.prm->constraint_At));
  else MI_TRY(P->apply(P, b.r, b.v));
  hipLaunchKernelGGL(first ? &k_cg_dot_rv<true> : &k_cg_dot_rv<false>, dim3(pl.grid), dim3(kBlock), 0, ctx->stream, pl.n,
                     (const CgState *)(first ? b.st0 : b.st1), (const double *)b.r->d, (const double *)b.v->d, b.p->d,
                     ctx->partials_b);
  return MI_OK;
}

int stpcg_setup(mi_ctx *ctx, const StpcgPlan &pl, StpcgBufs &b) {
  hipStream_t st = ctx->stream;
  const int grid = pl.grid;
  {
    KScope ks(ctx, MI_K_CG_INIT);
    if (pl.init_fused) {
      DISPATCH_P(pl.dgp->p, hipLaunchKernelGGL(k_cg_init_dirgram<P>, dim3(grid), dim3(StBlk<P>::threads), 0, st, pl.dgp->n,
                                               (const double *)b.g->d, b.r->d, b.p->d, b.s_out->d, ctx->partials_b, b.dga));
    } else {
      DISPATCH_PRE(pl.pre, hipLaunchKernelGGL(k_cg_init<PRE>, dim3(grid), dim3(kBlock), 0, st, pl.n, (const double *)b.g->d,
                                              b.pred, b.r->d, b.vd, b.p->d, b.s_out->d, ctx->partials_b));
    }
  }
  if (pl.pre == PRE_EXTERNAL) MI_TRY(stpcg_precondition(ctx, pl, b, true));
  if (pl.dgp) {
    if (!pl.init_fused) MI_TRY(launch_dirgram(ctx, pl, b, b.p->d));
    if (pl.recur && !pl.gdir_in_scalar_init) {
      MI_TRY(stpcg_allreduce(ctx, pl, ctx->partials2, grid, pl.gns, b.slots_g));
      hipLaunchKernelGGL(k_cg_gdir_init, dim3(1), dim3(kBlock), 0, st, (const double *)ctx->partials2, grid, pl.gns,
                         (const double *)b.slots_g, pl.sharded ? 1 : 0, b.dga.gdir);
    }
  }
  const CgSetup cfg{b.prm->Delta, b.prm->kappa_fgr, b.prm->theta, b.prm->epsilon,
                    (unsigned long long)b.prm->max_iterations};
  MI_TRY(stpcg_allreduce(ctx, pl, ctx->partials_b, grid, 1, b.slots_b));
  if (pl.sharded)
    hipLaunchKernelGGL(k_cg_scalar_init<true>, dim3(1), dim3(kBlock), 0, st, b.st0, cfg, (const double *)ctx->partials_b,
                       grid, (const double *)b.slots_b, ctx->status_dev, (const double *)nullptr, 0, 0, (double *)nullptr);
  else
    hipLaunchKernelGGL(k_cg_scalar_init<false>, dim3(1), dim3(kBlock), 0, st, b.st0, cfg, (const double *)ctx->partials_b,
                       grid, (const double *)b.slots_b, ctx->status_dev, (const double *)ctx->partials2, grid, pl.gns,
                       pl.gdir_in_scalar_init ? b.dga.gdir : (double *)nullptr);
  const hipError_t e = hipGetLastError();
  if (e != hipSuccess) return hip_fail(e, "stpcg init launch", __FILE__, __LINE__);
  return MI_OK;
}

int stpcg_reanchor(mi_ctx *ctx, const StpcgPlan &pl, StpcgBufs &b) {
  const int grid = pl.grid, gns = pl.gns;
  if (pl.dgp->p <= 4) {
    DISPATCH_P4(pl.dgp->p, hipLaunchKernelGGL(k_cg_dirgram2<P>, dim3(grid), dim3(kBlock), 0, ctx->stream, pl.dgp->n,
                                              (const CgState *)b.st0, (const double *)b.p->d, (const double *)b.r->d, b.dga));
    MI_TRY(stpcg_allreduce(ctx, pl, ctx->partials2, grid, 2 * gns, b.slots_g));
    launch_gdir_anchor(ctx, pl, b, b.dga.gdir + SLOT_GDIR_P, b.dga.gdir);
  } else {
    for (int which = 0; which < 2; ++which) {
      MI_TRY(launch_dirgram(ctx, pl, b, which == 0 ? b.p->d : b.r->d));
      MI_TRY(stpcg_allreduce(ctx, pl, ctx->partials2, grid, gns, b.slots_g));
      launch_gdir_anchor(ctx, pl, b, b.dga.gdir + (which == 0 ? SLOT_GDIR_P : 0), nullptr);
    }
  }
  return MI_OK;
}

int stpcg_operator(mi_ctx *ctx, const StpcgPlan &pl, StpcgBufs &b, int *nparts) {
  if (pl.dgp) return b.H->apply_dir(b.H, b.p, b.Hp, pl.recur ? -1 : pl.grid, nparts);
  if (b.H->apply_dots) return b.H->apply_dots(b.H, b.p, b.Hp, nparts);
  MI_TRY(b.H->apply(b.H, b.p, b.Hp));
  return launch_dot3_partials(ctx, pl.n, b.p->d, b.Hp->d, nparts);
}

int stpcg_step2(mi_ctx *ctx, const StpcgPlan &pl, StpcgBufs &b, size_t k, CgState **st_final) {
  CgState *cur = (k & 1) ? b.st1 : b.st0, *nxt = (k & 1) ? b.st0 : b.st1;
  int nparts = 0;
  ctx->cg_live = cur;
  ctx->twok_r = b.r->d;
  const int st_op = b.H->apply_dir(b.H, b.p, b.Hp, -2, &nparts);
  ctx->twok_r = nullptr;
  MI_TRY(st_op);
  KScope ks(ctx, MI_K_CG_UPDATE);
  hipLaunchKernelGGL(k_cg_step2<6>, dim3(pl.grid), dim3(kBlock), 0, ctx->stream, pl.n, pl.cc, (const CgState *)cur, nxt,
                     (const double *)ctx->partials, nparts, (const double *)b.Hp->d, b.r->d, b.p->d, b.s_out->d,
                     ctx->status_dev, b.tr, b.tcap, b.dga);
  *st_final = nxt;
  return MI_OK;
}

enum ObserverSays { OBS_GO_ON, OBS_STOP, OBS_LAST_PASS };
int stpcg_observe(mi_ctx *ctx, const StpcgPlan &pl, StpcgBufs &b, mi_stpcg_observer observer, void *observer_user,
                  int nparts, ObserverSays *says) {
  hipStream_t st = ctx->stream;
  ctx->host_syncs++;
  unsigned long long *flag = nullptr;
  const unsigned long long seq = poll_begin(ctx, &flag);
  {
    KScope ks(ctx, MI_K_CG_SCALAR_A);
    hipLaunchKernelGGL(k_cg_peek, dim3(1), dim3(kBlock), 0, st, pl.cc, (const CgState *)b.st0,
                       (const double *)ctx->partials, nparts, b.peek_dev, seq ? flag : (unsigned long long *)nullptr, seq);
  }
  hipError_t e = hipGetLastError();
  if (e != hipSuccess) return hip_fail(e, "stpcg observer peek launch", __FILE__, __LINE__);
  MI_TRY(poll_finish(ctx, seq, "stpcg observer peek"));
  const volatile unsigned long long *pk = reinterpret_cast<const volatile unsigned long long *>(ctx->cg_host);
  const int mode_in = (int)pk[0], mode_a = (int)pk[1];
  *says = OBS_STOP;
  if (mode_in == CG_DONE) return MI_OK;
  if (mode_a != CG_RUN) {
    *says = OBS_LAST_PASS;
    return MI_OK;
  }
  double alpha_k;
  const unsigned long long abits = pk[2];
  memcpy(&alpha_k, &abits, sizeof(alpha_k));
  ctx->cg_in_observer = true;
  const int stop = observer(observer_user, (size_t)pk[3], b.s_out, b.r, b.v ? b.v : b.r, b.p, alpha_k);
  ctx->cg_in_observer = false;
  *says = stop ? OBS_STOP : OBS_GO_ON;
  if (!stop) return MI_OK;
  hipLaunchKernelGGL(k_cg_user_stop, dim3(1), dim3(64), 0, st, b.st0, ctx->status_dev);
  e = hipGetLastError();
  if (e != hipSuccess) return hip_fail(e, "stpcg observer stop launch", __FILE__, __LINE__);
  return MI_OK;
}

int stpcg_astep(mi_ctx *ctx, const StpcgPlan &pl, StpcgBufs &b, size_t k, int nparts) {
  const bool sigma_later = pl.defer && (k & 1);
  FoldArgs fold_a;
  if (pl.folded) fold_a = comm_fold_next(ctx);
  else MI_TRY(stpcg_allreduce(ctx, pl, ctx->partials, nparts, pl.kc, pl.recur ? b.slots_g : b.slots_a));
  KScope ks(ctx, MI_K_CG_UPDATE);
  if (!pl.recur) {
    DISPATCH_PRE(pl.pre, launch_cg_update(pl.sharded    ? &k_cg_update<PRE, true, 3, NoFold>
                                          : sigma_later ? &k_cg_update_ns<PRE, false, 3, NoFold>
                                                        : &k_cg_update<PRE, false, 3, NoFold>,
                                          ctx, pl, b, nparts, NoFold{}));
  } else if (pl.kc > 16) {
    DISPATCH_KC_WIDE(pl.kc, launch_cg_update(pl.sharded    ? &k_cg_update<PRE_NONE, true, KC, NoFold>
                                             : sigma_later ? &k_cg_update_ns<PRE_NONE, false, KC, NoFold>
                                                           : &k_cg_update<PRE_NONE, false, KC, NoFold>,
                                             ctx, pl, b, nparts, NoFold{}));
  } else if (pl.folded) {
    DISPATCH_KC(pl.kc, launch_cg_update(&k_cg_update_s80<PRE_NONE, false, KC, FoldArgs>, ctx, pl, b, nparts, fold_a));
  } else {
    DISPATCH_KC(pl.kc, launch_cg_update(pl.sharded    ? &k_cg_update_s80<PRE_NONE, true, KC, NoFold>
                                        : sigma_later ? cg_update_recur_kernel<false, KC>()
                                                      : cg_update_recur_kernel<true, KC>(),
                                        ctx, pl, b, nparts, NoFold{}));
  }
  return MI_OK;
}

int stpcg_bstep(mi_ctx *ctx, const StpcgPlan &pl, StpcgBufs &b, size_t k) {
  hipStream_t st = ctx->stream;
  const mi_dirgram *dgp = pl.dgp;
  const int grid = pl.grid;
  if (pl.folded) {
    const FoldArgs fold_b = comm_fold_next(ctx);
    FoldPush fp{fold_b, HaloPush{}};
    const bool push = dgp->halo_A && k + 1 < b.prm->max_iterations &&
                      comm_halo_fold_next(ctx, dgp->halo_A, dgp->p, b.p->d, &fp.h);
    KScope ks(ctx, MI_K_CG_PUPDATE);
    if (push) launch_cg_pupdate(&k_cg_pupdate_s80<false, 0, FoldPush>, ctx, pl, b, fp);
    else launch_cg_pupdate(&k_cg_pupdate_s80<false, 0, FoldArgs>, ctx, pl, b, fold_b);
  } else if (pl.sharded) {
    MI_TRY(reduce_rows_allreduce(ctx, ctx->partials_b, grid, 1, b.slots_b));
    if (b.rprime) MI_TRY(comm_rprime_exchange(ctx, dgp->halo_A, dgp->p, b.r->d, nullptr, 0));
    KScope ks(ctx, MI_K_CG_PUPDATE);
    DISPATCH_SP(pl.sp, launch_cg_pupdate(cg_pupdate_kernel<true, SP>(), ctx, pl, b, NoFold{}));
  } else {
    if (pl.rows && b.rprime) MI_TRY(comm_rprime_exchange(ctx, dgp->halo_A, dgp->p, b.r->d, ctx->partials_b, 1));
    else if (pl.rows) MI_TRY(comm_allreduce_rows(ctx, ctx->partials_b, 1));
    KScope ks(ctx, MI_K_CG_PUPDATE);
    if (pl.early) {
      hipLaunchKernelGGL(k_cg_pupdate_early, dim3(grid), dim3(kBlock), 0, st, pl.n, pl.cc, (const CgState *)b.st1, b.st0,
                         (const double *)ctx->partials_b, grid, (const double *)b.vd, b.p->d, b.s_out->d, ctx->status_dev,
                         b.tr, b.tcap, b.dga);
    } else if (pl.defer && ((k & 1) || k + 1 < b.prm->max_iterations)) {
      hipLaunchKernelGGL((k & 1) ? &k_cg_pupdate_ds<true> : &k_cg_pupdate_ds<false>, dim3(grid), dim3(kBlock), 0, st,
                         pl.n, pl.cc, (const CgState *)b.st1, b.st0, (const double *)ctx->partials_b, grid,
                         (const double *)b.vd, (const double *)b.p->d, b.p2->d, b.s_out->d, ctx->status_dev, b.tr,
                         b.tcap, b.dga);
      std::swap(b.p, b.p2);
    } else {
      DISPATCH_SP(pl.sp, launch_cg_pupdate(cg_pupdate_kernel<false, SP>(), ctx, pl, b, NoFold{}));
    }
  }
  if (b.rprime && (pl.sharded || pl.rows)) {
    const double *hr = nullptr;
    double *hp = nullptr;
    size_t cnt = 0;
    comm_rprime_buffers(ctx, dgp->halo_A, dgp->p, &hr, &hp, &cnt);
    if (cnt) {
      const int hg = (int)std::max<size_t>(1, std::min<size_t>((cnt + 255) / 256, 512));
      hipLaunchKernelGGL(k_halo_dir, dim3(hg), dim3(256), 0, st, (const CgState *)b.st0, hr, hp, cnt);
    }
    comm_rprime_mark(ctx, dgp->halo_A, dgp->p, b.p->d);
  }
  return MI_OK;
}

int stpcg_result_from_host(mi_ctx *ctx, mi_stpcg_result *result) {
  int ipc_err = 0;
  (void)mi_comm_ipc_error(ctx, &ipc_err);
  if (ipc_err) {
    set_error("a wait in the peer-memory exchange layer timed out: the result of this solve is invalid");
    return MI_ERR_COMM;
  }
  const CgState &f = *ctx->cg_host;
  result->update_step_M_norm = f.M_norm;
  result->num_iterations = (size_t)f.k;
  result->exit_reason = f.exit_reason;
  result->rv_final = f.rv;
  return precon_fail_check(ctx, result);
}

int stpcg_readback(mi_ctx *ctx, const StpcgPlan &pl, const StpcgBufs &b, const CgState *st_final, mi_stpcg_trace *trace,
                   mi_stpcg_result *result) {
  hipStream_t st = ctx->stream;
  const mi_precon *P = b.P;
  const bool tracing = trace && trace->cap;
  *precon_fail_host(ctx) = 0.0;
  if (b.prm->defer_result && !tracing && !pl.observed) {
    hipError_t e = hipSuccess;
    ctx->cg_deferred_seq = result_to_host(ctx, st_final, P);
    if (!ctx->cg_deferred_seq) {
      if (!ctx->cg_deferred_ev) e = hipEventCreateWithFlags(&ctx->cg_deferred_ev, hipEventDisableTiming);
      if (e == hipSuccess) e = hipMemcpyAsync(ctx->cg_host, st_final, sizeof(CgState), hipMemcpyDeviceToHost, st);
      if (e == hipSuccess && P && P->fail_word)
        e = hipMemcpyAsync(precon_fail_host(ctx), P->fail_word, sizeof(double), hipMemcpyDeviceToHost, st);
      if (e == hipSuccess) e = hipEventRecord(ctx->cg_deferred_ev, st);
    }
    if (e != hipSuccess) return hip_fail(e, "stpcg deferred read-back", __FILE__, __LINE__);
    ctx->cg_deferred = true;
    ctx->cg_deferred_hvp = result->hvp_calls;
    result->update_step_M_norm = result->rv_final = 0;
    result->num_iterations = 0, result->exit_reason = -1, result->precon_status = 0;
    return MI_OK;
  }
  ctx->host_syncs++;
  if (const unsigned long long seq = result_to_host(ctx, st_final, P)) {
    MI_TRY(poll_finish(ctx, seq, "stpcg read-back"));
  } else {
    hipError_t e = hipMemcpyAsync(ctx->cg_host, st_final, sizeof(CgState), hipMemcpyDeviceToHost, st);
    if (e == hipSuccess && P && P->fail_word)
      e = hipMemcpyAsync(precon_fail_host(ctx), P->fail_word, sizeof(double), hipMemcpyDeviceToHost, st);
    if (e == hipSuccess) e = hipStreamSynchronize(st);
    if (e != hipSuccess) return hip_fail(e, "stpcg read-back", __FILE__, __LINE__);
  }
  MI_TRY(stpcg_result_from_host(ctx, result));
  if (tracing) {
    const size_t len = result->num_iterations < trace->cap ? result->num_iterations : trace->cap;
    trace->len = len;
    double *dst[4] = {trace->alpha, trace->beta, trace->kappa, trace->rv};
    for (int c = 0; c < 4; ++c)
      if (dst[c] && len) {
        const hipError_t e = hipMemcpy(dst[c], ctx->trace_dev + (size_t)c * b.tcap, len * sizeof(double),
                                       hipMemcpyDeviceToHost);
        if (e != hipSuccess) return hip_fail(e, "stpcg trace copy", __FILE__, __LINE__);
      }
  }
  return MI_OK;
}

int stpcg_solve(mi_ctx *ctx, const mi_vec *g, mi_op *H, mi_precon *P, const mi_stpcg_params *prm,
                mi_stpcg_observer observer, void *observer_user, mi_vec *s_out, mi_stpcg_result *result,
                mi_stpcg_trace *trace) {
  MI_REQUIRE(ctx && g && H && prm && s_out && result, "null argument");
  MI_REQUIRE(g->ctx == ctx && s_out->ctx == ctx && H->ctx == ctx, "objects belong to another context");
  MI_REQUIRE(g->n == s_out->n && g->n == H->n, "dimension mismatch: g %zu, s %zu, H %zu", g->n,
             s_out->n, H->n);
  MI_REQUIRE(g->d != s_out->d, "g and s_out must not alias");
  MI_REQUIRE(!ctx->cg_in_observer, "a solve was started on this context from inside an STPCG observer");
  const bool observed = observer != nullptr;
  if (observed) {
    const char *why = nullptr;
    if (mi_stpcg_observer_available(ctx, &why) != MI_OK) {
      set_error("mi_stpcg_observed declined: %s", why);
      return MI_DECLINED;
    }
  }
  touch(s_out);
  ctx->fusion.fused_stpcg_solves++;
  MI_REQUIRE(!P || (P->ctx == ctx && P->n == g->n), "preconditioner dimension/context mismatch");
  MI_REQUIRE(!prm->constraint_At || (P && P->apply_project),
             "constraint_At needs a constraint preconditioner (mi_precon_create_constraint)");
  MI_REQUIRE(!(P && P->kind == 3 && ctx->world_size > 1),
             "the constraint preconditioner is single-rank: its reductions are not completed across ranks");
  MI_REQUIRE(prm->Delta > 0, "Trust-region radius (Delta) must be a positive real value");
  MI_REQUIRE(prm->kappa_fgr >= 0 && prm->kappa_fgr < 1,
             "Target fractional reduction of the gradient norm (kappa_fgr) must be a real value in "
             "the range [0,1)");
  MI_REQUIRE(prm->theta >= 0 && prm->theta <= 1,
             "Target superlinear convergence rate (theta) must be a real value in the range [0,1]");
  MI_REQUIRE(prm->epsilon > 0 && prm->epsilon < 1,
             "Relative norm tolerance for declaring a vector to lie in the kernel of H (epsilon) "
             "should be a small positive number in the range (0,1)");

  RangeScope range("mi_stpcg");
  comm_halo_fold_drop(ctx);
  StpcgPlan plan;
  MI_TRY(stpcg_plan(ctx, H, P, prm, g->n, observed, plan));
  const StpcgPlan &pl = plan;
  StpcgBufs b(ctx);
  if (pl.recur && !pl.folded && pl.dgp->halo_A) MI_TRY(comm_rprime_prepare(ctx, pl.dgp->halo_A, &b.rprime));
  if (P && P->fail_word) MI_HIP(hipMemsetAsync(P->fail_word, 0, sizeof(double), ctx->stream));
  MI_TRY(stpcg_bufs(ctx, pl, g, H, P, prm, s_out, trace, b));
  ctx->cg_deferred = false;
  ctx->cg_deferred_seq = 0;
  ctx->epoch++;
  ctx->status->word = 0;
  ctx->status->epoch = ctx->epoch;
  ctx->cg_live = b.st0;
  MI_TRY(stpcg_setup(ctx, pl, b));

  CgState *st_final = b.st0;
  size_t hvp = 0;
  for (size_t k = 0; k < prm->max_iterations; ++k) {
    uint64_t w = ctx->status->word;
    while (!observed && !(w & 1) && k > (w >> 1) + (uint64_t)pl.run_ahead) {
      cpu_relax();
      w = ctx->status->word;
    }
    if (w & 1) {
      if (!pl.lockstep || k >= (w >> 1) + (uint64_t)pl.run_ahead) break;
    }
    if (pl.reanchor && k > 0 && k % (size_t)pl.reanchor == 0) MI_TRY(stpcg_reanchor(ctx, pl, b));
    if (pl.twok) {
      MI_TRY(stpcg_step2(ctx, pl, b, k, &st_final));
      ++hvp;
      continue;
    }
    int nparts = 0;
    MI_TRY(stpcg_operator(ctx, pl, b, &nparts));
    ++hvp;
    ObserverSays says = OBS_GO_ON;
    if (observed) MI_TRY(stpcg_observe(ctx, pl, b, observer, observer_user, nparts, &says));
    if (says == OBS_STOP) break;
    MI_TRY(stpcg_astep(ctx, pl, b, k, nparts));
    if (pl.pre == PRE_EXTERNAL) MI_TRY(stpcg_precondition(ctx, pl, b, false));
    MI_TRY(stpcg_bstep(ctx, pl, b, k));
    if (says == OBS_LAST_PASS) break;
  }
  result->hvp_calls = hvp;
  comm_halo_fold_drop(ctx);
  MI_TRY(stpcg_readback(ctx, pl, b, st_final, trace, result));
  b.ok = true;
  return MI_OK;
}

}

extern "C" {

int mi_stpcg_collect(mi_ctx *ctx, mi_stpcg_result *result) {
  MI_REQUIRE(ctx && result, "null argument");
  MI_REQUIRE(ctx->cg_deferred, "mi_stpcg_collect: no deferred solve is pending on this context");
  ctx->cg_deferred = false;
  if (ctx->cg_deferred_seq) {
    const unsigned long long seq = ctx->cg_deferred_seq;
    ctx->cg_deferred_seq = 0;
    if (__atomic_load_n(ctx->poll_flag, __ATOMIC_ACQUIRE) < seq) {
      ctx->host_syncs++;
      MI_TRY(poll_finish(ctx, seq, "stpcg deferred read-back"));
    }
  } else {
    hipError_t e = hipEventQuery(ctx->cg_deferred_ev);
    if (e == hipErrorNotReady) {
      e = hipEventSynchronize(ctx->cg_deferred_ev);
      ctx->host_syncs++;
    }
    if (e != hipSuccess) return hip_fail(e, "stpcg deferred read-back", __FILE__, __LINE__);
  }
  result->hvp_calls = ctx->cg_deferred_hvp;
  return stpcg_result_from_host(ctx, result);
}

int mi_stpcg_observer_available(mi_ctx *ctx, const char **why) {
  MI_REQUIRE(ctx, "null argument");
  const char *w = nullptr;
  if (ctx->cfg.no_fused_observer) w = "MI355OPT_NO_FUSED_OBSERVER is set";
  else if (ctx->world_size > 1) w = "the context is one of several ranks";
  else if (ctx->force_lockstep) w = "MI355OPT_FORCE_LOCKSTEP is set";
  else if (slot_mode(ctx) || rows_mode(ctx)) w = "the context completes its reductions through an exchange layer";
  if (why) *why = w ? w : "";
  return w ? MI_DECLINED : MI_OK;
}

int mi_stpcg(mi_ctx *ctx, const mi_vec *g, mi_op *H, mi_precon *P, const mi_stpcg_params *prm, mi_vec *s_out,
             mi_stpcg_result *result, mi_stpcg_trace *trace) {
  return stpcg_solve(ctx, g, H, P, prm, nullptr, nullptr, s_out, result, trace);
}

int mi_stpcg_observed(mi_ctx *ctx, const mi_vec *g, mi_op *H, mi_precon *P, const mi_stpcg_params *prm,
                      mi_stpcg_observer fn, void *user, mi_vec *s_out, mi_stpcg_result *result, mi_stpcg_trace *trace) {
  MI_REQUIRE(fn, "mi_stpcg_observed: null observer (mi_stpcg is the solve without one)");
  return stpcg_solve(ctx, g, H, P, prm, fn, user, s_out, result, trace);
}

}
```

optimization_amd/csrc/stpcg_kernels.inc:

```

template <int PRE, bool FROM_SLOTS, int KC = 3, class FOLD = NoFold>
__global__ __launch_bounds__(kBlock) CG_KERNEL_ATTR void CG_UPDATE_NAME(size_t n, CgConst cc, const CgState *__restrict__ st_in,
                                                      CgState *__restrict__ st_out,
                                                      const double *__restrict__ partials_a, int nparts_a,
                                                      const double *__restrict__ slots,
                                                      const double *__restrict__ p,
                                                      const double *__restrict__ Hp,
                                                      const double *__restrict__ pre,
                                                      double *__restrict__ s, double *__restrict__ r,
                                                      double *__restrict__ v,
                                                      double *__restrict__ partials_b, DirGramArgs dg,
                                                      FOLD fold) {
  __shared__ double lds[3 * (kWaves + 1)];
  static_assert(KC >= 3 && KC <= 3 * (kWaves + 1), "3 curvature dots + at most 36 Gram components (p <= 8)");
  CgState cs = load_state(st_in);
  if (cs.mode == CG_DONE) {
    if (blockIdx.x == 0 && threadIdx.x == 0) store_state(st_out, cs);
    return;
  }
  FOLD_STAMP(0);
  const size_t n2 = n >> 1, stride = (size_t)gridDim.x * kBlock;
  const size_t i0 = (size_t)blockIdx.x * kBlock + threadIdx.x;
  auto next_of = [&](size_t i_) -> size_t { return i_ + stride; };
  const size_t ifirst = i0;
  double2 hv0 = make_double2(0, 0), rv0 = hv0;
  constexpr bool kFolded = !std::is_same<FOLD, NoFold>::value;
  auto prefetch_now = [&] {
    if (PRE != PRE_BLOCK3 && ifirst < n2) {
      hv0 = reinterpret_cast<const double2 *>(Hp)[ifirst];
      rv0 = reinterpret_cast<double2 *>(r)[ifirst];
    }
  };
  auto prefetch = [&] {
    if (kFolded && threadIdx.x < 64) return;
    prefetch_now();
  };
  double d[KC];
  if (FROM_SLOTS) {
    prefetch_now();
#pragma unroll
    for (int i = 0; i < KC; ++i) d[i] = slots[i];
  } else {
    reduce_rows<KC>(partials_a, nparts_a, d, lds, prefetch);
    fold_maybe<KC>(d, fold, lds);
    if (kFolded && threadIdx.x < 64) prefetch_now();
    if (!kFolded) FOLD_STAMP(1);
  }
  step_a(cs, cc, d[0], d[1], d[2]);
  if (!kFolded) FOLD_STAMP(5);
  if (blockIdx.x == 0 && threadIdx.x == 0) {
    store_state(st_out, cs);
    if (KC > 3 && cs.mode == CG_RUN) {
#pragma unroll
      for (int i = 0; i < KC - 3; ++i)
        if (i < dg.ns) dg.gdir[i] = dg.gdir[i] + cs.alpha * d[3 + i];
    }
  }

  const int mode = cs.mode;
  double acc[1] = {0};
  if (mode == CG_APPLY_SIGMA) {
    if (!CG_UPDATE_SIGMA) return;
    const double sigma = cs.sigma;
    for (size_t i = i0; i < n2; i += stride) {
      const double2 pv = reinterpret_cast<const double2 *>(p)[i];
      double2 sv = reinterpret_cast<double2 *>(s)[i];
      sv.x += sigma * pv.x; sv.y += sigma * pv.y;
      reinterpret_cast<double2 *>(s)[i] = sv;
    }
    if ((n & 1) && blockIdx.x == 0 && threadIdx.x == 0) s[n - 1] += sigma * p[n - 1];
    return;
  }
  if (mode == CG_KERNEL_PENDING) {
    for (size_t i = i0; i < n2; i += stride) {
      const double2 pv = reinterpret_cast<const double2 *>(p)[i];
      const double2 rv = reinterpret_cast<const double2 *>(r)[i];
      acc[0] += pv.x * rv.x; acc[0] += pv.y * rv.y;
    }
    if ((n & 1) && blockIdx.x == 0 && threadIdx.x == 0) acc[0] += p[n - 1] * r[n - 1];
  } else {
    const double alpha = cs.alpha;
    if (PRE == PRE_BLOCK3) {
      const size_t nb = n / 3;
      for (size_t b = i0; b < nb; b += stride) {
        double rr[3];
#pragma unroll
        for (int c = 0; c < 3; ++c) {
          const size_t i = 3 * b + c;
          rr[c] = r[i] + alpha * Hp[i];
          r[i] = rr[c];
        }
        const double *M = pre + 9 * b;
#pragma unroll
        for (int c = 0; c < 3; ++c) {
          const double vv = M[3 * c] * rr[0] + M[3 * c + 1] * rr[1] + M[3 * c + 2] * rr[2];
          v[3 * b + c] = vv;
          acc[0] += rr[c] * vv;
        }
      }
    } else {
      double2 hv = hv0, rv = rv0;
      for (size_t i = ifirst; i < n2;) {
        const size_t inext = next_of(i);
        double2 hn = hv, rn = rv;
        if (inext < n2) {
          hn = reinterpret_cast<const double2 *>(Hp)[inext];
          rn = reinterpret_cast<double2 *>(r)[inext];
        }
        rv.x += alpha * hv.x; rv.y += alpha * hv.y;
        reinterpret_cast<double2 *>(r)[i] = rv;
        if (PRE != PRE_EXTERNAL) {
          double2 vv = rv;
          if (PRE == PRE_DIAG) {
            const double2 dd = reinterpret_cast<const double2 *>(pre)[i];
            vv.x = dd.x * rv.x; vv.y = dd.y * rv.y;
            reinterpret_cast<double2 *>(v)[i] = vv;
          }
          acc[0] += rv.x * vv.x; acc[0] += rv.y * vv.y;
        }
        i = inext; hv = hn; rv = rn;
      }
      if ((n & 1) && blockIdx.x == 0 && threadIdx.x == 0) {
        const size_t i = n - 1;
        const double rv = r[i] + alpha * Hp[i];
        r[i] = rv;
        if (PRE != PRE_EXTERNAL) {
          double vv = rv;
          if (PRE == PRE_DIAG) { vv = pre[i] * rv; v[i] = vv; }
          acc[0] += rv * vv;
        }
      }
    }
    if (PRE == PRE_EXTERNAL) return;
  }
  block_partials_store<1>(acc, lds, partials_b);
  FOLD_STAMP(6);
}

template <bool FROM_SLOTS, int SP, class FOLD = NoFold>
__global__ __launch_bounds__(kBlock) CG_KERNEL_ATTR void CG_PUPDATE_NAME(size_t n, CgConst cc, const CgState *__restrict__ st_in,
                                                       CgState *__restrict__ st_out,
                                                       const double *__restrict__ partials_b, int nparts_b,
                                                       const double *__restrict__ slots,
                                                       const double *__restrict__ v,
                                                       double *__restrict__ p, double *__restrict__ s,
                                                       HostStatus *hs, double *__restrict__ trace,
                                                       size_t trace_cap, DirGramArgs dg, FOLD fold) {
  __shared__ double lds[DirGramLds<SP>::value];
  CgState cs = load_state(st_in);
  const bool leader = blockIdx.x == 0 && threadIdx.x == 0;
  if (cs.mode == CG_DONE) {
    if (leader) store_state(st_out, cs);
    return;
  }
  const int mode_in = cs.mode;
  const size_t n2 = n >> 1, stride = (size_t)gridDim.x * kBlock;
  const size_t i0 = (size_t)blockIdx.x * kBlock + threadIdx.x;
  const size_t tail0 = cc.rag0, per = cc.rag_per;
  const size_t irem = (threadIdx.x < per) ? tail0 + (size_t)blockIdx.x * per + threadIdx.x : n2;
  auto next_of = [&](size_t i_) -> size_t {
    const size_t j_ = i_ + stride;
    return j_ < tail0 ? j_ : ((i_ < tail0 && irem < n2) ? irem : n2);
  };
  const size_t ifirst = i0 < tail0 ? i0 : (irem < n2 ? irem : n2);
  double2 vv0 = make_double2(0, 0), pv0 = vv0, sv0 = vv0;
  constexpr int SPN = SP > 0 ? SP : 1;
  double rv0[SPN], rp0[SPN], rs0[SPN], rx0[SPN], ry0[SPN];
#pragma unroll
  for (int c = 0; c < SPN; ++c) { rv0[c] = 0; rp0[c] = 0; rs0[c] = 0; rx0[c] = 0; ry0[c] = 0; }
  auto prefetch_now = [&] {
    if (SP > 0) {
      if (mode_in == CG_RUN && i0 < n / SPN) {
#pragma unroll
        for (int c = 0; c < SPN; ++c) {
          rv0[c] = v[i0 * SPN + c];
          rp0[c] = p[i0 * SPN + c];
          rs0[c] = s[i0 * SPN + c];
          rx0[c] = dg.X[i0 * SPN + c];
          ry0[c] = dg.Y[i0 * SPN + c];
        }
      }
    } else if (ifirst < n2) {
      const size_t q0 = halo_phys(fold, ifirst);
      vv0 = reinterpret_cast<const double2 *>(v)[q0];
      pv0 = reinterpret_cast<double2 *>(p)[q0];
      sv0 = reinterpret_cast<double2 *>(s)[q0];
    }
  };
  double red[1] = {0};
  if (mode_in != CG_APPLY_SIGMA && !FROM_SLOTS) {
    reduce_rows<1>(partials_b, nparts_b, red, lds, prefetch_now);
    fold_maybe<1>(red, fold, lds);
  } else {
    prefetch_now();
    if (mode_in != CG_APPLY_SIGMA) red[0] = slots[0];
  }
  step_b(cs, cc, red[0]);
  cs.launches = cs.launches + 1;
  if (leader) {
    store_state(st_out, cs);
    if (mode_in == CG_RUN && trace && cs.k - 1 < trace_cap) {
      const size_t k = (size_t)(cs.k - 1);
      trace[k] = cs.alpha;
      trace[trace_cap + k] = cs.beta;
      trace[2 * trace_cap + k] = cs.kappa;
      trace[3 * trace_cap + k] = cs.rv;
    }
// ... 96 lines not shown
```

Baseline: 5831.

## Fuse Steihaug-CG setup into Stiefel gradient finish and specialize first iterations

Adds a lean setup path where the Stiefel RQ gradient-finish kernel also emits the residual norm partials and direction-Gram rows. CG then skips its separate init pass and copies of r/p from g. The first update and pupdate kernels read g directly, with sign flips in place of materialized r and p, which removes initialization memory traffic and launches per solve. This brings extra kernel variants, a setup record that must be validated against the gradient's serial and generation, and a debug/option surface.

```diff
diff --git a/include/mi355opt.h b/include/mi355opt.h
--- a/include/mi355opt.h
+++ b/include/mi355opt.h
@@ -302,6 +302,8 @@
 MI_API int mi_debug_window_runs(int ntiles, int max_wgs, int num_cu, size_t far_stride, int *bounds_out, int cap,
                                 int *nb_out);
 MI_API int mi_debug_stiefel_hess_form(int p, int gram_count, const size_t traits[9], const int switches[9], int out[14]);
+MI_API int mi_debug_stpcg_setup(const mi_ctx *ctx, int *kind);
+MI_API int mi_debug_stpcg_lean_setup(const int facts[13], int *lean);
 MI_API int mi_debug_set_rank(mi_ctx *ctx, int world_size, int rank);
 MI_API int mi_debug_csr_set_halo(mi_csr *A, int p, const double *halo_rows_host);
 MI_API int mi_debug_time_fused_apply(mi_op *op, const mi_vec *in, mi_vec *out, int reps, double *us_per_call);
diff --git a/optimization_amd/capi.py b/optimization_amd/capi.py
--- a/optimization_amd/capi.py
+++ b/optimization_amd/capi.py
@@ -227,6 +227,8 @@
         "mi_debug_so3n_info": [vp, c_size_p],
         "mi_debug_time_fused_apply": [vp, vp, vp, C.c_int, c_double_p],
         "mi_debug_set_rank": [vp, C.c_int, C.c_int],
+        "mi_debug_stpcg_setup": [vp, C.POINTER(C.c_int)],
+        "mi_debug_stpcg_lean_setup": [C.POINTER(C.c_int), C.POINTER(C.c_int)],
         "mi_debug_csr_set_halo": [vp, C.c_int, c_double_p],
         "mi_csr_create_sharded": [vp, C.c_size_t, C.c_size_t, C.c_size_t, C.c_size_t, c_int32_p,
                                   c_int64_p, c_double_p, c_size_p, C.POINTER(vp)],
@@ -275,6 +277,17 @@
     return list(out) if st == MI_OK else None
 
 
+STPCG_SETUPS = ("full", "lean", "none")
+LEAN_FACTS = ("recur", "init_fused", "gdir_in_scalar_init", "defer", "twok", "early", "observed", "one_context",
+              "no_lean_setup", "record_matches", "pre", "p", "max_iterations")
+
+
+def stpcg_lean_setup(**facts):
+    out = C.c_int(0)
+    check(load().mi_debug_stpcg_lean_setup((C.c_int * 13)(*[int(facts[k]) for k in LEAN_FACTS]), C.byref(out)))
+    return bool(out.value)
+
+
 def csr_shard_plan(n_global, world_size, rank, row_starts, col_global):
     L = load()
     L.mi_csr_shard_plan.restype = C.c_int
@@ -323,6 +336,11 @@
     def set_option(self, name, value):
         check(self.L.mi_ctx_set_option(self.h, name.encode(), int(value)))
         return self
+
+    def stpcg_setup(self):
+        k = C.c_int(0)
+        check(self.L.mi_debug_stpcg_setup(self.h, C.byref(k)))
+        return STPCG_SETUPS[k.value]
 
     def sync_count(self):
         n = C.c_size_t(0)
diff --git a/optimization_amd/csrc/context.hip b/optimization_amd/csrc/context.hip
--- a/optimization_amd/csrc/context.hip
+++ b/optimization_amd/csrc/context.hip
@@ -228,6 +228,7 @@
 OPT_BOOL(opt_so3_no_rquat, cfg.so3_no_rquat)
 OPT_BOOL(opt_early_s, cfg.early_s)
 OPT_BOOL(opt_defer_s, cfg.defer_s)
+OPT_BOOL(opt_no_lean_setup, cfg.no_lean_setup)
 OPT_BOOL(opt_no_fused_observer, cfg.no_fused_observer)
 OPT_BOOL(opt_no_fused_lsqr_observer, cfg.no_fused_lsqr_observer)
 OPT_BOOL(opt_no_update_pair, cfg.no_update_pair)
@@ -272,7 +273,7 @@
     {"WORDS16", opt_words16}, {"NO_SPMM_STREAM", opt_no_spmm_stream}, {"NO_SPMM_WIN", opt_no_spmm_win},
     {"NO_SPMM_SWEEP", opt_no_spmm_sweep}, {"SWEEP_ZSEGS", opt_sweep_zsegs, true},
     {"NO_ZERO_COPY", opt_no_zero_copy}, {"NO_POLLED_SYNC", opt_no_polled_sync}, {"WIDE_QUAD", opt_wide_quad, true}, {"WIDE_WINDOW", opt_wide_window, true},
-    {"NO_UPDATE_MFMA", opt_no_update_mfma}, {"HALO_RPRIME", opt_halo_rprime}, {"NO_GRAM_HALF", opt_no_gram_half}, {"SO3_NO_QUAT", opt_so3_no_quat}, {"SO3_NO_RQUAT", opt_so3_no_rquat}, {"EARLY_S", opt_early_s}, {"DEFER_S", opt_defer_s}, {"NO_FUSED_OBSERVER", opt_no_fused_observer}, {"NO_FUSED_LSQR_OBSERVER", opt_no_fused_lsqr_observer}, {"NO_UPDATE_PAIR", opt_no_update_pair}, {"TWO_KERNEL_STEP", opt_two_kernel_step}, {"SO3_SORT_NBR", opt_so3_sort_nbr, true},
+    {"NO_UPDATE_MFMA", opt_no_update_mfma}, {"HALO_RPRIME", opt_halo_rprime}, {"NO_GRAM_HALF", opt_no_gram_half}, {"SO3_NO_QUAT", opt_so3_no_quat}, {"SO3_NO_RQUAT", opt_so3_no_rquat}, {"EARLY_S", opt_early_s}, {"DEFER_S", opt_defer_s}, {"NO_LEAN_SETUP", opt_no_lean_setup}, {"NO_FUSED_OBSERVER", opt_no_fused_observer}, {"NO_FUSED_LSQR_OBSERVER", opt_no_fused_lsqr_observer}, {"NO_UPDATE_PAIR", opt_no_update_pair}, {"TWO_KERNEL_STEP", opt_two_kernel_step}, {"SO3_SORT_NBR", opt_so3_sort_nbr, true},
     {"WARN_GENERIC", opt_warn_generic}, {"TALL_PROLOGUE", opt_tall_prologue}, {"REANCHOR", opt_reanchor, true},
 };
 bool option_value(const OptionDesc &o, const char *e, long *v) {
diff --git a/optimization_amd/csrc/mi_internal.h b/optimization_amd/csrc/mi_internal.h
--- a/optimization_amd/csrc/mi_internal.h
+++ b/optimization_amd/csrc/mi_internal.h
@@ -135,6 +135,7 @@
   bool so3_no_rquat = false;
   bool so3_no_quat = false;
   int so3_sort_nbr = 0;
+  bool no_lean_setup = false;
   bool tall_prologue = false;
 };
 
@@ -169,6 +170,7 @@
   mi::CgState *cg_host = nullptr;
   const double *twok_r = nullptr;
   const mi::CgState *cg_live = nullptr;
+  int cg_last_setup = 0;
   hipEvent_t cg_deferred_ev = nullptr;
   bool cg_deferred = false;
   size_t cg_deferred_hvp = 0;
@@ -522,6 +524,21 @@
   bool borrowed = false;
 };
 
+struct mi_setup_record {
+  bool valid = false;
+  const mi_vec *g = nullptr;
+  const double *g_d = nullptr;
+  uint64_t serial = 0, gen = 0;
+  size_t n = 0;
+  int p = 0, grid = 0;
+  const double *X = nullptr, *Y = nullptr, *S = nullptr;
+  double *rv_rows = nullptr;
+  double *gram_rows = nullptr;
+};
+namespace mi {
+enum StpcgSetupKind { STPCG_SETUP_FULL = 0, STPCG_SETUP_LEAN = 1, STPCG_SETUP_NONE = 2 };
+}
+
 struct mi_dirgram {
   int p = 0;
   size_t n = 0;
@@ -530,6 +547,7 @@
   const double *S = nullptr;
   const struct mi_csr *halo_A = nullptr;
   bool twok = false;
+  const mi_setup_record *setup = nullptr;
 };
 
 struct mi_precon {
diff --git a/optimization_amd/csrc/stiefel.hip b/optimization_amd/csrc/stiefel.hip
--- a/optimization_amd/csrc/stiefel.hip
+++ b/optimization_amd/csrc/stiefel.hip
@@ -1019,6 +1019,81 @@
   if (DOTS) block_partials_store_w<3, NW>(a, lds, partials);
 }
 
+template <int P>
+__global__ __launch_bounds__(StBlk<P>::threads) void k_st_finish_setup(size_t n, const double *__restrict__ X,
+                                                                       const double *__restrict__ Z,
+                                                                       const double *__restrict__ gram_partials, int count,
+                                                                       double *__restrict__ M_out, double *__restrict__ out,
+                                                                       double *__restrict__ rv_rows,
+                                                                       double *__restrict__ g_rows) {
+  static_assert(P >= 1 && P <= 4, "narrow rows");
+  constexpr int BLK = StBlk<P>::threads, NW = StBlk<P>::waves;
+  __shared__ double lds[SymIdx<P>::NS * (kWaves + 1) + 3 * kWaves];
+  const size_t stride = (size_t)gridDim.x * BLK;
+  const size_t row0 = (size_t)blockIdx.x * BLK + threadIdx.x;
+  double x[P], z[P];
+#pragma unroll
+  for (int c = 0; c < P; ++c) { x[c] = 0; z[c] = 0; }
+  if (row0 < n) {
+#pragma unroll
+    for (int c = 0; c < P; ++c) {
+      x[c] = X[row0 * P + c];
+      z[c] = Z[row0 * P + c];
+    }
+  }
+  double Mm[P * P];
+  load_sym<P, false>(gram_partials, count, nullptr, Mm, lds);
+  if (M_out && blockIdx.x == 0 && threadIdx.x == 0) {
+#pragma unroll
+    for (int i = 0; i < P * P; ++i) M_out[i] = Mm[i];
+  }
+  double G[P * P], acc[1] = {0};
+#pragma unroll
+  for (int i = 0; i < P * P; ++i) G[i] = 0;
+  for (size_t row = row0; row < n;) {
+    const size_t rnext = row + stride;
+    double xn[P], zn[P];
+#pragma unroll
+    for (int c = 0; c < P; ++c) { xn[c] = x[c]; zn[c] = z[c]; }
+    if (rnext < n) {
+#pragma unroll
+      for (int c = 0; c < P; ++c) {
+        xn[c] = X[rnext * P + c];
+        zn[c] = Z[rnext * P + c];
+      }
+    }
+    double gv[P], pv[P];
+#pragma unroll
+    for (int b = 0; b < P; ++b) {
+      double t = 0;
+#pragma unroll
+      for (int aa = 0; aa < P; ++aa) t += x[aa] * Mm[aa * P + b];
+      const double o = z[b] - t;
+      out[row * P + b] = o;
+      gv[b] = o;
+    }
+#pragma unroll
+    for (int c = 0; c < P; ++c) {
+      pv[c] = -gv[c];
+      acc[0] += gv[c] * gv[c];
+    }
+#pragma unroll
+    for (int b = 0; b < P; ++b) {
+      double t = 0;
+#pragma unroll
+      for (int a = 0; a < P; ++a) t += pv[a] * Mm[a * P + b];
+#pragma unroll
+      for (int a = 0; a < P; ++a) G[a * P + b] += z[a] * pv[b] - x[a] * t;
+    }
+    row = rnext;
+#pragma unroll
+    for (int c = 0; c < P; ++c) { x[c] = xn[c]; z[c] = zn[c]; }
+  }
+  store_sym_partials<P>(G, lds, g_rows);
+  __syncthreads();
+  block_partials_store_w<1, NW>(acc, lds, rv_rows);
+}
+
 template <int P, bool FROM_SLOTS>
 __global__ __launch_bounds__(StBlk<P>::threads) void k_st_polar(size_t n, double *__restrict__ Y,
                                                      const double *__restrict__ gram_partials, int count,
@@ -1117,6 +1192,17 @@
   return MI_OK;
 }
 
+int launch_finish_setup(mi_ctx *ctx, size_t n, int p, const double *X, const double *Z, int count, double *M_out,
+                        double *out, const mi_setup_record &rec, int *grid_out) {
+  const int grid = grid_for(ctx, n * (size_t)p, 4);
+  KScope ks(ctx, MI_K_STIEFEL_FINISH_DOTS);
+  DISPATCH_P4(p, hipLaunchKernelGGL(k_st_finish_setup<P>, dim3(grid), dim3(StBlk<P>::threads), 0, ctx->stream, n, X, Z,
+                                    (const double *)ctx->partials2, count, M_out, out, rec.rv_rows, rec.gram_rows));
+  *grid_out = grid;
+  MI_HIP(hipGetLastError());
+  return MI_OK;
+}
+
 int check_np(mi_ctx *ctx, size_t n, int p, const mi_vec *a, const mi_vec *b, const mi_vec *c) {
   MI_REQUIRE(ctx, "ctx is null");
   MI_REQUIRE(p >= 1 && p <= kMaxPTall, "p must be in [1,%d], got %d", kMaxPTall, p);
@@ -1141,6 +1227,7 @@
   mi_vec *Z;
   mi_vec *Y;
   mi_dirgram dg;
+  mi_setup_record setup;
   mi_op hess;
   const mi_vec *X;
   uint64_t X_serial = 0;
@@ -1531,6 +1618,10 @@
   MI_HIP(hipMemsetAsync(q->S_dev, 0, kMaxPTall * kMaxPTall * sizeof(double), ctx->stream));
   MI_TRY(mi_vec_create(ctx, n * (size_t)p, &q->Z));
   MI_TRY(mi_vec_create(ctx, n * (size_t)p, &q->Y));
+  if (p <= 4) {
+    MI_HIP(hipMalloc((void **)&q->setup.rv_rows, (size_t)(1 + nsym(p)) * kMaxRows * sizeof(double)));
+    q->setup.gram_rows = q->setup.rv_rows + kMaxRows;
+  }
   q->hess.ctx = ctx;
   q->hess.n = n * (size_t)p;
   q->hess.apply = rq_apply;
@@ -1547,6 +1638,7 @@
   (void)hipStreamSynchronize(q->ctx->stream);
   (void)hipFree(q->S_dev);
   (void)hipFree(q->S_next);
+  (void)hipFree(q->setup.rv_rows);
   mi_vec_destroy(q->Z);
   mi_vec_destroy(q->Y);
   mi_vec_destroy(q->Y_next);
@@ -1590,17 +1682,28 @@
 int mi_stiefel_rq_model(mi_stiefel_rq *q, const mi_vec *X, mi_vec *grad, mi_op **hess) {
   MI_REQUIRE(q && X && grad, "null argument");
   MI_TRY(check_np(q->ctx, q->n, q->p, X, grad, nullptr));
-  int count = 0;
+  int count = 0, setup_grid = 0;
   touch(grad);
+  q->setup.valid = false;
   if (q->is_trial(X)) {
     std::swap(q->Y, q->Y_next);
     std::swap(q->S_dev, q->S_next);
     MI_TRY(mi_vec_copy(grad, q->grad_next));
   } else {
     MI_TRY(launch_spmm_gram(q->ctx, q->A, q->p, nullptr, X->d, X->d, nullptr, q->Y->d, &count));
-    MI_TRY(launch_finish(q->ctx, q->n, q->p, nullptr, X->d, q->Y->d, nullptr, count, q->S_dev, grad->d, false,
-                         nullptr));
-  }
+    mi_ctx *ctx = q->ctx;
+    if (q->setup.rv_rows && !ctx->cfg.no_lean_setup && !ctx->uniform_grid && !slot_mode(ctx) && !rows_mode(ctx)) {
+      MI_TRY(launch_finish_setup(ctx, q->n, q->p, X->d, q->Y->d, count, q->S_dev, grad->d, q->setup, &setup_grid));
+    } else {
+      MI_TRY(launch_finish(q->ctx, q->n, q->p, nullptr, X->d, q->Y->d, nullptr, count, q->S_dev, grad->d, false,
+                           nullptr));
+    }
+  }
+  q->setup.valid = setup_grid > 0;
+  q->setup.g = grad, q->setup.g_d = grad->d, q->setup.serial = grad->serial, q->setup.gen = gen_of(grad);
+  q->setup.n = q->n, q->setup.p = q->p, q->setup.grid = setup_grid;
+  q->setup.X = X->d, q->setup.Y = q->Y->d, q->setup.S = q->S_dev;
+  q->dg.setup = &q->setup;
   q->trial_X = nullptr;
   q->X = X;
   q->X_serial = X->serial;
@@ -1629,6 +1732,7 @@
   MI_TRY(check_np(q->ctx, q->n, q->p, X_trial, nullptr, nullptr));
   mi_ctx *ctx = q->ctx;
   ctx->fusion.fused_trial_steps++;
+  q->setup.valid = false;
   const size_t N = q->n * (size_t)q->p;
   if (!q->Y_next) {
     MI_TRY(mi_vec_create(ctx, N, &q->Y_next));
@@ -1692,6 +1796,7 @@
   MI_TRY(check_np(q->ctx, q->n, q->p, X_trial, nullptr, nullptr));
   mi_ctx *ctx = q->ctx;
   ctx->fusion.fused_trial_steps++;
+  q->setup.valid = false;
   const size_t N = q->n * (size_t)q->p;
   if (!q->Y_next) {
     MI_TRY(mi_vec_create(ctx, N, &q->Y_next));
diff --git a/optimization_amd/csrc/stpcg.hip b/optimization_amd/csrc/stpcg.hip
--- a/optimization_amd/csrc/stpcg.hip
+++ b/optimization_amd/csrc/stpcg.hip
@@ -203,7 +203,7 @@
 }
 
 __device__ __forceinline__ void gdir_from_rows(const double *__restrict__ partials, int count, int gns,
-                                               double *__restrict__ gdir) {
+                                               double *__restrict__ gdir, bool first_g = false) {
   const int lane = threadIdx.x & 63;
   for (int w = threadIdx.x >> 6; w < gns; w += kWaves) {
     const double *src = partials + (size_t)w * kMaxRows;
@@ -218,7 +218,7 @@
     for (int j = 0; j < kMaxRows / 64; ++j) v += t[j];
     v = wave_reduce_sum(v);
     if (lane == 0) {
-      gdir[SLOT_GDIR_P + w] = v;
+      gdir[SLOT_GDIR_P + w] = first_g ? -v : v;
       gdir[w] = -v;
     }
   }
@@ -248,7 +248,7 @@
   unsigned long long max_iterations;
 };
 
-template <bool FROM_SLOTS>
+template <bool FROM_SLOTS, bool FIRST_G = false>
 __global__ __launch_bounds__(kBlock) void k_cg_scalar_init(CgState *st, CgSetup cfg,
                                                            const double *partials, int nparts,
                                                            const double *slots, HostStatus *hs,
@@ -256,7 +256,7 @@
                                                            double *__restrict__ gdir) {
 #pragma clang fp contract(off)
   __shared__ double lds[kWaves + 1];
-  if (gdir) gdir_from_rows(gpartials, gcount, gns, gdir);
+  if (gdir) gdir_from_rows(gpartials, gcount, gns, gdir, FIRST_G);
   double red[1];
   if (FROM_SLOTS) red[0] = slots[0];
   else reduce_rows<1>(partials, nparts, red, lds);
@@ -315,6 +315,7 @@
 
 #define CG_KERNEL_ATTR
 #define CG_UPDATE_SIGMA 1
+#define CG_FIRST 0
 #define CG_UPDATE_NAME k_cg_update
 #define CG_PUPDATE_NAME k_cg_pupdate
 #include "stpcg_kernels.inc"
@@ -345,6 +346,25 @@
 #undef CG_UPDATE_NAME
 #undef CG_PUPDATE_NAME
 #undef CG_UPDATE_SIGMA
+#undef CG_FIRST
+#define CG_FIRST 1
+#define CG_UPDATE_SIGMA 1
+#define CG_KERNEL_ATTR
+#define CG_UPDATE_NAME k_cg_first_update
+#define CG_PUPDATE_NAME k_cg_first_dir_unused
+#include "stpcg_kernels.inc"
+#undef CG_KERNEL_ATTR
+#undef CG_UPDATE_NAME
+#undef CG_PUPDATE_NAME
+#define CG_KERNEL_ATTR __attribute__((amdgpu_num_sgpr(80), amdgpu_waves_per_eu(8, 8)))
+#define CG_UPDATE_NAME k_cg_first_update_s80
+#define CG_PUPDATE_NAME k_cg_first_dir_s80_unused
+#include "stpcg_kernels.inc"
+#undef CG_KERNEL_ATTR
+#undef CG_UPDATE_NAME
+#undef CG_PUPDATE_NAME
+#undef CG_UPDATE_SIGMA
+#undef CG_FIRST
 
 template <class F>
 __device__ __forceinline__ void reduce_rows_1x512(const double *__restrict__ partials, int count, double &out, double *lds,
@@ -581,6 +601,125 @@
 }
 
 
+template <bool FLUSH>
+__global__ __launch_bounds__(kBlock) __attribute__((amdgpu_waves_per_eu(8, 8))) void k_cg_first_pupdate(
+    size_t n, CgConst cc, const CgState *__restrict__ st_in, CgState *__restrict__ st_out,
+    const double *__restrict__ partials_b, int nparts_b, const double *__restrict__ v, const double *__restrict__ pc,
+    const double *__restrict__ g, double *__restrict__ px, double *__restrict__ s, HostStatus *hs,
+    double *__restrict__ trace, size_t trace_cap, DirGramArgs dg) {
+  __shared__ double lds[kWaves + 1];
+  CgState cs = load_state(st_in);
+  const bool leader = blockIdx.x == 0 && threadIdx.x == 0;
+  if (cs.mode == CG_DONE) {
+    if (leader) store_state(st_out, cs);
+    return;
+  }
+  const int mode_in = cs.mode;
+  const size_t n2 = n >> 1, stride = (size_t)gridDim.x * kBlock;
+  const size_t i0 = (size_t)blockIdx.x * kBlock + threadIdx.x;
+  const size_t tail0 = cc.rag0, per = cc.rag_per;
+  const size_t irem = (threadIdx.x < per) ? tail0 + (size_t)blockIdx.x * per + threadIdx.x : n2;
+  auto next_of = [&](size_t i_) -> size_t {
+    const size_t j_ = i_ + stride;
+    return j_ < tail0 ? j_ : ((i_ < tail0 && irem < n2) ? irem : n2);
+  };
+  const size_t ifirst = i0 < tail0 ? i0 : (irem < n2 ? irem : n2);
+  double2 vv0 = make_double2(0, 0), pv0 = vv0, gv0 = vv0;
+  auto prefetch_now = [&] {
+    if (ifirst < n2) {
+      vv0 = reinterpret_cast<const double2 *>(v)[ifirst];
+      gv0 = reinterpret_cast<const double2 *>(g)[ifirst];
+      if (FLUSH) pv0 = reinterpret_cast<const double2 *>(pc)[ifirst];
+    }
+  };
+  double red[1] = {0};
+  if (mode_in != CG_APPLY_SIGMA) reduce_rows<1>(partials_b, nparts_b, red, lds, prefetch_now);
+  else prefetch_now();
+  step_b(cs, cc, red[0]);
+  cs.launches = cs.launches + 1;
+  const bool dir = mode_in == CG_RUN && cs.mode == CG_RUN;
+  if (leader) {
+    store_state(st_out, cs);
+    if (!FLUSH && dir) st_out->alpha_prev = cs.alpha;
+    if (mode_in == CG_RUN && trace && cs.k - 1 < trace_cap) {
+      const size_t k = (size_t)(cs.k - 1);
+      trace[k] = cs.alpha;
+      trace[trace_cap + k] = cs.beta;
+      trace[2 * trace_cap + k] = cs.kappa;
+      trace[3 * trace_cap + k] = cs.rv;
+    }
+    publish(hs, cs.launches, cs.mode == CG_DONE);
+    if (dg.gdir && dir) {
+      for (int i = 0; i < dg.ns; ++i) {
+        const double gp = FLUSH ? dg.gdir[SLOT_GDIR_P + i] : -dg.gdir[SLOT_GDIR_P + i];
+        dg.gdir[SLOT_GDIR_P + i] = -dg.gdir[i] + cs.beta * gp;
+      }
+    }
+  }
+  const double beta = cs.beta;
+  if (FLUSH) {
+    const double alpha_old = st_out->alpha_prev, alpha = mode_in == CG_RUN ? cs.alpha : cs.sigma;
+    double2 vv = vv0, pv = pv0, gv = gv0;
+    for (size_t i = ifirst; i < n2;) {
+      const size_t inext = next_of(i);
+      double2 vn = vv, pn = pv, gn = gv;
+      if (inext < n2) {
+        vn = reinterpret_cast<const double2 *>(v)[inext];
+        pn = reinterpret_cast<const double2 *>(pc)[inext];
+        gn = reinterpret_cast<const double2 *>(g)[inext];
+      }
+      const double2 ov = make_double2(-gv.x, -gv.y);
+      double2 sv = make_double2(0 * gv.x, 0 * gv.y);
+      sv.x = sv.x + alpha_old * ov.x; sv.y = sv.y + alpha_old * ov.y;
+      sv.x = sv.x + alpha * pv.x; sv.y = sv.y + alpha * pv.y;
+      reinterpret_cast<double2 *>(s)[i] = sv;
+      if (dir) {
+        pv.x = -vv.x + beta * pv.x; pv.y = -vv.y + beta * pv.y;
+        reinterpret_cast<double2 *>(px)[i] = pv;
+      }
+      i = inext; vv = vn; pv = pn; gv = gn;
+    }
+    if ((n & 1) && leader) {
+      const double gl = g[n - 1], ol = -gl;
+      double sl = 0 * gl;
+      sl = sl + alpha_old * ol;
+      sl = sl + alpha * pc[n - 1];
+      s[n - 1] = sl;
+      if (dir) px[n - 1] = -v[n - 1] + beta * pc[n - 1];
+    }
+  } else if (dir) {
+    double2 vv = vv0, gv = gv0;
+    for (size_t i = ifirst; i < n2;) {
+      const size_t inext = next_of(i);
+      double2 vn = vv, gn = gv;
+      if (inext < n2) {
+        vn = reinterpret_cast<const double2 *>(v)[inext];
+        gn = reinterpret_cast<const double2 *>(g)[inext];
+      }
+      double2 pv = make_double2(-gv.x, -gv.y);
+      pv.x = -vv.x + beta * pv.x; pv.y = -vv.y + beta * pv.y;
+      reinterpret_cast<double2 *>(px)[i] = pv;
+      i = inext; vv = vn; gv = gn;
+    }
+    if ((n & 1) && leader) px[n - 1] = -v[n - 1] + beta * (-g[n - 1]);
+  } else if (mode_in != CG_APPLY_SIGMA) {
+    const double alpha = mode_in == CG_RUN ? cs.alpha : cs.sigma;
+    for (size_t i = i0; i < n2; i += stride) {
+      const double2 gv = reinterpret_cast<const double2 *>(g)[i];
+      const double2 pv = make_double2(-gv.x, -gv.y);
+      double2 sv = make_double2(0 * gv.x, 0 * gv.y);
+      sv.x = sv.x + alpha * pv.x; sv.y = sv.y + alpha * pv.y;
+      reinterpret_cast<double2 *>(s)[i] = sv;
+    }
+    if ((n & 1) && leader) {
+      const double gl = g[n - 1], pl = -gl;
+      double sl = 0 * gl;
+      sl = sl + alpha * pl;
+      s[n - 1] = sl;
+    }
+  }
+}
+
 template <int NS>
 __global__ __launch_bounds__(kBlock) void k_cg_step2(size_t n, CgConst cc, const CgState *__restrict__ st_in,
                                                      CgState *__restrict__ st_out, const double *__restrict__ partials_a,
@@ -942,6 +1081,11 @@
   else if constexpr (KC == 16) return &k_cg_update_ns_s80<PRE_NONE, false, KC, NoFold>;
   else return &k_cg_update_ns<PRE_NONE, false, KC, NoFold>;
 }
+template <int KC>
+auto cg_update_first_kernel() {
+  if constexpr (KC == 16) return &k_cg_first_update_s80<PRE_NONE, false, KC, NoFold>;
+  else return &k_cg_first_update<PRE_NONE, false, KC, NoFold>;
+}
 template <bool FS, int SP>
 auto cg_pupdate_kernel() {
   if constexpr (SP == 1 || (FS && SP == 0)) return &k_cg_pupdate_s80<FS, SP, NoFold>;
@@ -952,13 +1096,30 @@
   size_t n;
   bool observed, sharded, rows, lockstep, recur, folded, init_fused, gdir_in_scalar_init;
   bool twok, early, defer;
+  bool lean_setup;
   int pre, run_ahead, grid, gns, sp, kc, reanchor;
   const mi_dirgram *dgp;
   CgConst cc;
 };
 
-int stpcg_plan(const mi_ctx *ctx, const mi_op *H, const mi_precon *P, const mi_stpcg_params *prm, size_t n,
-               bool observed, StpcgPlan &pl) {
+struct StpcgLeanFacts {
+  bool recur, init_fused, gdir_in_scalar_init, defer, twok, early, observed, one_context, no_lean_setup, record_matches;
+  int pre, p;
+  unsigned long long max_iterations;
+};
+bool stpcg_lean_scope(const StpcgLeanFacts &f) {
+  return f.recur && f.init_fused && f.gdir_in_scalar_init && f.defer && !f.twok && !f.early && !f.observed &&
+         f.pre == PRE_NONE && f.one_context && f.p >= 1 && f.p <= 4 && f.max_iterations >= 2 && !f.no_lean_setup &&
+         f.record_matches;
+}
+bool setup_record_matches(const mi_setup_record *rec, const mi_vec *g, const mi_dirgram *dgp, int grid) {
+  return rec && dgp && g && rec->valid && rec->g == g && rec->g_d == g->d && rec->serial == g->serial &&
+         rec->gen == gen_of(g) && rec->n == dgp->n && rec->p == dgp->p && rec->X == dgp->X && rec->Y == dgp->Y &&
+         rec->S == dgp->S && rec->grid == grid && rec->rv_rows && rec->gram_rows;
+}
+
+int stpcg_plan(const mi_ctx *ctx, const mi_op *H, const mi_precon *P, const mi_stpcg_params *prm, const mi_vec *g,
+               size_t n, bool observed, StpcgPlan &pl) {
   pl.n = n;
   pl.observed = observed;
   pl.pre = !P ? PRE_NONE : (P->kind == 1 ? PRE_DIAG : (P->kind == 2 ? PRE_BLOCK3 : PRE_EXTERNAL));
@@ -990,6 +1151,11 @@
   pl.defer = !pl.sharded && !pl.rows && !pl.lockstep && !pl.twok && pl.sp == 0 && !pl.early && ctx->cfg.defer_s &&
              !observed;
   pl.reanchor = (pl.recur && !pl.twok && ctx->cfg.reanchor > 0) ? ctx->cfg.reanchor : 0;
+  pl.lean_setup = stpcg_lean_scope(
+      {pl.recur, pl.init_fused, pl.gdir_in_scalar_init, pl.defer, pl.twok, pl.early, observed,
+       !pl.sharded && !pl.rows && !pl.lockstep, ctx->cfg.no_lean_setup,
+       setup_record_matches(pl.dgp ? pl.dgp->setup : nullptr, g, pl.dgp, pl.grid), pl.pre, pl.dgp ? pl.dgp->p : 0,
+       (unsigned long long)prm->max_iterations});
   return MI_OK;
 }
 
@@ -1092,6 +1258,17 @@
 int stpcg_setup(mi_ctx *ctx, const StpcgPlan &pl, StpcgBufs &b) {
   hipStream_t st = ctx->stream;
   const int grid = pl.grid;
+  if (pl.lean_setup) {
+    const mi_setup_record *rec = pl.dgp->setup;
+    const CgSetup cfg{b.prm->Delta, b.prm->kappa_fgr, b.prm->theta, b.prm->epsilon,
+                      (unsigned long long)b.prm->max_iterations};
+    hipLaunchKernelGGL((k_cg_scalar_init<false, true>), dim3(1), dim3(kBlock), 0, st, b.st0, cfg,
+                       (const double *)rec->rv_rows, grid, (const double *)b.slots_b, ctx->status_dev,
+                       (const double *)rec->gram_rows, grid, pl.gns, b.dga.gdir);
+    const hipError_t e = hipGetLastError();
+    if (e != hipSuccess) return hip_fail(e, "stpcg init launch", __FILE__, __LINE__);
+    return MI_OK;
+  }
   {
     KScope ks(ctx, MI_K_CG_INIT);
     if (pl.init_fused) {
@@ -1143,7 +1320,8 @@
   return MI_OK;
 }
 
-int stpcg_operator(mi_ctx *ctx, const StpcgPlan &pl, StpcgBufs &b, int *nparts) {
+int stpcg_operator(mi_ctx *ctx, const StpcgPlan &pl, StpcgBufs &b, size_t k, int *nparts) {
+  if (pl.lean_setup && k == 0) return b.H->apply_dir(b.H, b.g, b.Hp, -1, nparts);
   if (pl.dgp) return b.H->apply_dir(b.H, b.p, b.Hp, pl.recur ? -1 : pl.grid, nparts);
   if (b.H->apply_dots) return b.H->apply_dots(b.H, b.p, b.Hp, nparts);
   MI_TRY(b.H->apply(b.H, b.p, b.Hp));
@@ -1209,6 +1387,14 @@
   if (pl.folded) fold_a = comm_fold_next(ctx);
   else MI_TRY(stpcg_allreduce(ctx, pl, ctx->partials, nparts, pl.kc, pl.recur ? b.slots_g : b.slots_a));
   KScope ks(ctx, MI_K_CG_UPDATE);
+  if (pl.lean_setup && k == 0) {
+    DISPATCH_KC(pl.kc, hipLaunchKernelGGL(cg_update_first_kernel<KC>(), dim3(pl.grid), dim3(kBlock), 0, ctx->stream, pl.n,
+                                          pl.cc, (const CgState *)b.st0, b.st1, (const double *)ctx->partials, nparts,
+                                          (const double *)b.slots_g, (const double *)b.g->d, (const double *)b.Hp->d,
+                                          (const double *)b.g->d, b.s_out->d, b.r->d, b.vd, ctx->partials_b, b.dga,
+                                          NoFold{}));
+    return MI_OK;
+  }
   if (!pl.recur) {
     DISPATCH_PRE(pl.pre, launch_cg_update(pl.sharded    ? &k_cg_update<PRE, true, 3, NoFold>
                                           : sigma_later ? &k_cg_update_ns<PRE, false, 3, NoFold>
@@ -1255,6 +1441,12 @@
       hipLaunchKernelGGL(k_cg_pupdate_early, dim3(grid), dim3(kBlock), 0, st, pl.n, pl.cc, (const CgState *)b.st1, b.st0,
                          (const double *)ctx->partials_b, grid, (const double *)b.vd, b.p->d, b.s_out->d, ctx->status_dev,
                          b.tr, b.tcap, b.dga);
+    } else if (pl.lean_setup && k < 2) {
+      hipLaunchKernelGGL(k ? &k_cg_first_pupdate<true> : &k_cg_first_pupdate<false>, dim3(grid), dim3(kBlock), 0, st, pl.n,
+                         pl.cc, (const CgState *)b.st1, b.st0, (const double *)ctx->partials_b, grid, (const double *)b.vd,
+                         (const double *)b.p->d, (const double *)b.g->d, b.p2->d, b.s_out->d, ctx->status_dev, b.tr, b.tcap,
+                         b.dga);
+      std::swap(b.p, b.p2);
     } else if (pl.defer && ((k & 1) || k + 1 < b.prm->max_iterations)) {
       hipLaunchKernelGGL((k & 1) ? &k_cg_pupdate_ds<true> : &k_cg_pupdate_ds<false>, dim3(grid), dim3(kBlock), 0, st,
                          pl.n, pl.cc, (const CgState *)b.st1, b.st0, (const double *)ctx->partials_b, grid,
@@ -1379,7 +1571,7 @@
   RangeScope range("mi_stpcg");
   comm_halo_fold_drop(ctx);
   StpcgPlan plan;
-  MI_TRY(stpcg_plan(ctx, H, P, prm, g->n, observed, plan));
+  MI_TRY(stpcg_plan(ctx, H, P, prm, g, g->n, observed, plan));
   const StpcgPlan &pl = plan;
   StpcgBufs b(ctx);
   if (pl.recur && !pl.folded && pl.dgp->halo_A) MI_TRY(comm_rprime_prepare(ctx, pl.dgp->halo_A, &b.rprime));
@@ -1391,6 +1583,7 @@
   ctx->status->word = 0;
   ctx->status->epoch = ctx->epoch;
   ctx->cg_live = b.st0;
+  ctx->cg_last_setup = pl.lean_setup ? STPCG_SETUP_NONE : STPCG_SETUP_FULL;
   MI_TRY(stpcg_setup(ctx, pl, b));
 
   CgState *st_final = b.st0;
@@ -1411,7 +1604,7 @@
       continue;
     }
     int nparts = 0;
-    MI_TRY(stpcg_operator(ctx, pl, b, &nparts));
+    MI_TRY(stpcg_operator(ctx, pl, b, k, &nparts));
     ++hvp;
     ObserverSays says = OBS_GO_ON;
     if (observed) MI_TRY(stpcg_observe(ctx, pl, b, observer, observer_user, nparts, &says));
@@ -1431,6 +1624,20 @@
 }
 
 extern "C" {
+
+int mi_debug_stpcg_setup(const mi_ctx *ctx, int *kind) {
+  MI_REQUIRE(ctx && kind, "null argument");
+  *kind = ctx->cg_last_setup;
+  return MI_OK;
+}
+
+int mi_debug_stpcg_lean_setup(const int f[13], int *lean) {
+  MI_REQUIRE(f && lean, "null argument");
+  *lean = stpcg_lean_scope({f[0] != 0, f[1] != 0, f[2] != 0, f[3] != 0, f[4] != 0, f[5] != 0, f[6] != 0, f[7] != 0,
+                            f[8] != 0, f[9] != 0, f[10], f[11], (unsigned long long)(f[12] < 0 ? 0 : f[12])})
+              ? 1 : 0;
+  return MI_OK;
+}
 
 int mi_stpcg_collect(mi_ctx *ctx, mi_stpcg_result *result) {
   MI_REQUIRE(ctx && result, "null argument");
diff --git a/optimization_amd/csrc/stpcg_kernels.inc b/optimization_amd/csrc/stpcg_kernels.inc
--- a/optimization_amd/csrc/stpcg_kernels.inc
+++ b/optimization_amd/csrc/stpcg_kernels.inc
@@ -16,6 +16,13 @@
   CgState cs = load_state(st_in);
   if (cs.mode == CG_DONE) {
     if (blockIdx.x == 0 && threadIdx.x == 0) store_state(st_out, cs);
+#if CG_FIRST
+    for (size_t i = (size_t)blockIdx.x * kBlock + threadIdx.x; i < (n >> 1); i += (size_t)gridDim.x * kBlock) {
+      const double2 gv = reinterpret_cast<const double2 *>(pre)[i];
+      reinterpret_cast<double2 *>(s)[i] = make_double2(0 * gv.x, 0 * gv.y);
+    }
+    if ((n & 1) && blockIdx.x == 0 && threadIdx.x == 0) s[n - 1] = 0 * pre[n - 1];
+#endif
     return;
   }
   FOLD_STAMP(0);
@@ -28,7 +35,11 @@
   auto prefetch_now = [&] {
     if (PRE != PRE_BLOCK3 && ifirst < n2) {
       hv0 = reinterpret_cast<const double2 *>(Hp)[ifirst];
+#if CG_FIRST
+      rv0 = reinterpret_cast<const double2 *>(pre)[ifirst];
+#else
       rv0 = reinterpret_cast<double2 *>(r)[ifirst];
+#endif
     }
   };
   auto prefetch = [&] {
@@ -46,6 +57,10 @@
     if (kFolded && threadIdx.x < 64) prefetch_now();
     if (!kFolded) FOLD_STAMP(1);
   }
+#if CG_FIRST
+#pragma unroll
+  for (int i = 3; i < KC; ++i) d[i] = -d[i];
+#endif
   step_a(cs, cc, d[0], d[1], d[2]);
   if (!kFolded) FOLD_STAMP(5);
   if (blockIdx.x == 0 && threadIdx.x == 0) {
@@ -63,21 +78,45 @@
     if (!CG_UPDATE_SIGMA) return;
     const double sigma = cs.sigma;
     for (size_t i = i0; i < n2; i += stride) {
+#if CG_FIRST
+      const double2 gv = reinterpret_cast<const double2 *>(pre)[i];
+      const double2 pv = make_double2(-gv.x, -gv.y);
+      double2 sv = make_double2(0 * gv.x, 0 * gv.y);
+#else
       const double2 pv = reinterpret_cast<const double2 *>(p)[i];
       double2 sv = reinterpret_cast<double2 *>(s)[i];
+#endif
       sv.x += sigma * pv.x; sv.y += sigma * pv.y;
       reinterpret_cast<double2 *>(s)[i] = sv;
     }
+#if CG_FIRST
+    if ((n & 1) && blockIdx.x == 0 && threadIdx.x == 0) {
+      const double gl = pre[n - 1], pl = -gl;
+      double sl = 0 * gl;
+      sl += sigma * pl;
+      s[n - 1] = sl;
+    }
+#else
     if ((n & 1) && blockIdx.x == 0 && threadIdx.x == 0) s[n - 1] += sigma * p[n - 1];
+#endif
     return;
   }
   if (mode == CG_KERNEL_PENDING) {
     for (size_t i = i0; i < n2; i += stride) {
+#if CG_FIRST
+      const double2 rv = reinterpret_cast<const double2 *>(pre)[i];
+      const double2 pv = make_double2(-rv.x, -rv.y);
+#else
       const double2 pv = reinterpret_cast<const double2 *>(p)[i];
       const double2 rv = reinterpret_cast<const double2 *>(r)[i];
+#endif
       acc[0] += pv.x * rv.x; acc[0] += pv.y * rv.y;
     }
+#if CG_FIRST
+    if ((n & 1) && blockIdx.x == 0 && threadIdx.x == 0) acc[0] += (-pre[n - 1]) * pre[n - 1];
+#else
     if ((n & 1) && blockIdx.x == 0 && threadIdx.x == 0) acc[0] += p[n - 1] * r[n - 1];
+#endif
   } else {
     const double alpha = cs.alpha;
     if (PRE == PRE_BLOCK3) {
@@ -105,8 +144,15 @@
         double2 hn = hv, rn = rv;
         if (inext < n2) {
           hn = reinterpret_cast<const double2 *>(Hp)[inext];
+#if CG_FIRST
+          rn = reinterpret_cast<const double2 *>(pre)[inext];
+#else
           rn = reinterpret_cast<double2 *>(r)[inext];
-        }
+#endif
+        }
+#if CG_FIRST
+        hv.x = -hv.x; hv.y = -hv.y;
+#endif
         rv.x += alpha * hv.x; rv.y += alpha * hv.y;
         reinterpret_cast<double2 *>(r)[i] = rv;
         if (PRE != PRE_EXTERNAL) {
@@ -122,7 +168,11 @@
       }
       if ((n & 1) && blockIdx.x == 0 && threadIdx.x == 0) {
         const size_t i = n - 1;
+#if CG_FIRST
+        const double rv = pre[i] + alpha * (-Hp[i]);
+#else
         const double rv = r[i] + alpha * Hp[i];
+#endif
         r[i] = rv;
         if (PRE != PRE_EXTERNAL) {
           double vv = rv;
```

Result: no change. 5875, median of 6 (+0.8%).
